# nv-tlabs/3dgrut

Measured on NVIDIA H100. Metric: train frames/sec (fwd+bwd render), higher is better.
Workload: dtype f32

## Files before the change

### 3dgrut_b200/csrc/gut_api.cu

```cuda
#include <cuda_runtime.h>

#include <algorithm>
#include <cmath>
#include <cstdarg>
#include <cstdio>
#include <cstdlib>
#include <cstring>
#include <new>
#include <string>

#include "gut_common.cuh"

using namespace gutb200;

namespace {


struct Quat {
    float w, x, y, z;
};
struct Mat3 {
    float m[3][3];
};
struct Pose {
    float t[3];
    Quat q;
};

Mat3 to_mat3(const Quat& q) {
    const float qxx = q.x * q.x, qyy = q.y * q.y, qzz = q.z * q.z;
    const float qxz = q.x * q.z, qxy = q.x * q.y, qyz = q.y * q.z;
    const float qwx = q.w * q.x, qwy = q.w * q.y, qwz = q.w * q.z;
    Mat3 r;
    r.m[0][0] = 1.f - 2.f * (qyy + qzz); r.m[0][1] = 2.f * (qxy + qwz); r.m[0][2] = 2.f * (qxz - qwy);
    r.m[1][0] = 2.f * (qxy - qwz); r.m[1][1] = 1.f - 2.f * (qxx + qzz); r.m[1][2] = 2.f * (qyz + qwx);
    r.m[2][0] = 2.f * (qxz + qwy); r.m[2][1] = 2.f * (qyz - qwx); r.m[2][2] = 1.f - 2.f * (qxx + qyy);
    return r;
}

Quat to_quat(const Mat3& a) {
    const float(*m)[3] = a.m;
    Quat q;
    const float tr = m[0][0] + m[1][1] + m[2][2];
    if (tr > 0.f) {
        const float S = std::sqrt(tr + 1.f) * 2.f;
        q = {0.25f * S, (m[1][2] - m[2][1]) / S, (m[2][0] - m[0][2]) / S, (m[0][1] - m[1][0]) / S};
    } else if (m[0][0] > m[1][1] && m[0][0] > m[2][2]) {
        const float S = std::sqrt(1.f + m[0][0] - m[1][1] - m[2][2]) * 2.f;
        q = {(m[1][2] - m[2][1]) / S, 0.25f * S, (m[1][0] + m[0][1]) / S, (m[2][0] + m[0][2]) / S};
    } else if (m[1][1] > m[2][2]) {
        const float S = std::sqrt(1.f + m[1][1] - m[0][0] - m[2][2]) * 2.f;
        q = {(m[2][0] - m[0][2]) / S, (m[1][0] + m[0][1]) / S, 0.25f * S, (m[2][1] + m[1][2]) / S};
    } else {
        const float S = std::sqrt(1.f + m[2][2] - m[0][0] - m[1][1]) * 2.f;
        q = {(m[0][1] - m[1][0]) / S, (m[2][0] + m[0][2]) / S, (m[2][1] + m[1][2]) / S, 0.25f * S};
    }
    return q;
}

Quat slerp(const Quat& x, const Quat& y, float t) {
    Quat z = y;
    float c = (x.w * y.w + x.x * y.x) + (x.y * y.y + x.z * y.z);
    if (c < 0.f) {
        z = {-y.w, -y.x, -y.y, -y.z};
        c = -c;
    }
    if (c > 1.f - 1.1920929e-07f) {
        const float a = 1.f - t;
        return {x.w * a + z.w * t, x.x * a + z.x * t, x.y * a + z.y * t, x.z * a + z.z * t};
    }
    const float ang = std::acos(c);
    const float s0 = std::sin((1.f - t) * ang), s1 = std::sin(t * ang), sd = std::sin(ang);
    return {(s0 * x.w + s1 * z.w) / sd, (s0 * x.x + s1 * z.x) / sd, (s0 * x.y + s1 * z.y) / sd, (s0 * x.z + s1 * z.z) / sd};
}

Pose pose_from7(const float* p) { return Pose{{p[0], p[1], p[2]}, Quat{p[6], p[3], p[4], p[5]}}; }

Pose pose_inverse(const Pose& p) {
    const Mat3 r = to_mat3(p.q);
    Mat3 inv;
    for (int c = 0; c < 3; ++c)
        for (int k = 0; k < 3; ++k) inv.m[c][k] = r.m[k][c];
    Pose o;
    o.q = to_quat(inv);
    for (int j = 0; j < 3; ++j) {
        float acc = 0.f;
        acc += (-1.0f * inv.m[0][j]) * p.t[0];
        acc += (-1.0f * inv.m[1][j]) * p.t[1];
        acc += (-1.0f * inv.m[2][j]) * p.t[2];
        o.t[j] = acc;
    }
    return o;
}

void pose_cols(const Pose& p, float cols[12]) {
    const Mat3 r = to_mat3(p.q);
    for (int c = 0; c < 3; ++c)
        for (int k = 0; k < 3; ++k) cols[c * 3 + k] = r.m[c][k];
    cols[9] = p.t[0];
    cols[10] = p.t[1];
    cols[11] = p.t[2];
}


struct DeviceBuffer {
    void* ptr = nullptr;
    size_t bytes = 0;
    cudaError_t reserve(size_t want, cudaStream_t s, bool zero = false) {
        if (want <= bytes) return cudaSuccess;
        if (ptr) {
            cudaError_t e = cudaFreeAsync(ptr, s);
            if (e != cudaSuccess) return e;
            ptr = nullptr;
            bytes = 0;
        }
        const size_t padded = (want + (want >> 3) + 255) & ~size_t(255);
        cudaError_t e = cudaMallocAsync(&ptr, padded, s);
        if (e != cudaSuccess) return e;
        bytes = padded;
        if (zero) e = cudaMemsetAsync(ptr, 0, padded, s);
        return e;
    }
    void release() {
        if (ptr) cudaFree(ptr);
        ptr = nullptr;
        bytes = 0;
    }
    template <typename T>
    T* as() const { return static_cast<T*>(ptr); }
};

}

struct gutb200_ctx {
    gutb200_config cfg;
    int device = 0;
    std::string error;
    cudaStream_t own_stream = nullptr;

    DeviceBuffer tiles_count, proj, depth, rgb, grad_acc;
    DeviceBuffer keys64, keys64_alt, vals_out, hit_words;
    DeviceBuffer tile_hist, tile_fill, sub_base, ranges, tile_order, chunk_base, totals, scan_parts;
    cudaEvent_t ev_total = nullptr;
    gutb200_camera fwd_camera{};
    DeviceBuffer h_particles, h_sph, h_rays_o, h_rays_d, h_rgba, h_dist, h_hits, h_vis, h_drgba, h_ddist, h_dpart, h_dsph;
    uint32_t* pinned_total = nullptr;

    FrameCamera cam{};
    FrameConfig fcfg{};
    int64_t n = -1, num_isect = 0, num_tiles = 0;
    bool have_forward = false;
    bool fwd_nht = false;
    cudaStream_t fwd_stream = nullptr;

    cudaEvent_t ev[4] = {nullptr, nullptr, nullptr, nullptr};
    double fwd_ms = 0, bwd_ms = 0;
    int fwd_calls = 0, bwd_calls = 0;
    bool fwd_pending = false, bwd_pending = false;
    int64_t launches = 0;

    cudaEvent_t st_ev[8][2] = {};
    bool st_pending[8] = {};
    double st_ms[8] = {};
    int st_calls[8] = {};
};

namespace {

int fail(gutb200_ctx* c, const char* fmt, ...) {
    char buf[512];
    va_list ap;
    va_start(ap, fmt);
    vsnprintf(buf, sizeof(buf), fmt, ap);
    va_end(ap);
    if (c) c->error = buf;
    return 1;
}

#define GUT_CUDA(ctx, expr)                                                                             \
    do {                                                                                                \
        cudaError_t e__ = (expr);                                                                       \
        if (e__ != cudaSuccess) return fail(ctx, "%s failed: %s", #expr, cudaGetErrorString(e__));      \
    } while (0)

void fill_frame(gutb200_ctx* c, const gutb200_camera* cam) {
    FrameCamera& f = c->cam;
    f.width = cam->width;
    f.height = cam->height;
    f.grid_x = (cam->width + kTile - 1) / kTile;
    f.grid_y = (cam->height + kTile - 1) / kTile;
    f.fx = cam->focal[0]; f.fy = cam->focal[1];
    f.cx = cam->principal[0]; f.cy = cam->principal[1];
    memcpy(f.radial, cam->radial, sizeof(f.radial));
    memcpy(f.tangential, cam->tangential, sizeof(f.tangential));
    memcpy(f.thin_prism, cam->thin_prism, sizeof(f.thin_prism));
    f.has_distortion = 0;
    for (float v : cam->radial) f.has_distortion |= (v != 0.f);
    for (float v : cam->tangential) f.has_distortion |= (v != 0.f);
    for (float v : cam->thin_prism) f.has_distortion |= (v != 0.f);
    f.res_x = static_cast<float>(cam->width);
    f.res_y = static_cast<float>(cam->height);
    f.model = cam->model;
    f.max_angle = cam->max_angle;
    f.ft_reference_poly = cam->ftheta_reference_poly;
    memcpy(f.ft_bw, cam->ftheta_bw, sizeof(f.ft_bw));
    memcpy(f.ft_fw, cam->ftheta_fw, sizeof(f.ft_fw));
    memcpy(f.ft_cde, cam->ftheta_cde, sizeof(f.ft_cde));
    const Pose ps = pose_from7(cam->pose_start), pe = pose_from7(cam->pose_end);
    const Mat3 rs = to_mat3(ps.q);
    for (int cc = 0; cc < 3; ++cc)
        for (int k = 0; k < 3; ++k) f.rot_start[cc * 3 + k] = rs.m[cc][k];
    for (int k = 0; k < 3; ++k) f.t_start[k] = ps.t[k];
    f.rolling_shutter = cam->rolling_shutter;
    f.rs_iterations = c->cfg.n_rolling_shutter_iterations;
    f.q_start[0] = ps.q.w; f.q_start[1] = ps.q.x; f.q_start[2] = ps.q.y; f.q_start[3] = ps.q.z;
    f.q_end[0] = pe.q.w; f.q_end[1] = pe.q.x; f.q_end[2] = pe.q.y; f.q_end[3] = pe.q.z;
    for (int k = 0; k < 3; ++k) f.t_end[k] = pe.t[k];
    Pose mid;
    mid.q = slerp(ps.q, pe.q, 0.5f);
    for (int k = 0; k < 3; ++k) mid.t[k] = ps.t[k] * (1.f - 0.5f) + pe.t[k] * 0.5f;
    const Pose inv = pose_inverse(mid);
    pose_cols(mid, f.view);
    pose_cols(inv, f.s2w);
    for (int k = 0; k < 3; ++k) f.cam_pos[k] = inv.t[k];

    FrameConfig& g = c->fcfg;
    const gutb200_config& s = c->cfg;
    g.kernel_degree = s.kernel_degree;
    g.min_kernel_density = s.min_kernel_density;
    g.min_alpha = s.min_alpha;
    g.max_alpha = s.max_alpha;
    g.min_transmittance = s.min_transmittance;
    g.ut_delta = s.ut_delta;
    g.ut_margin = s.ut_margin;
    const float D = 3.f;
    const float lambda = s.ut_alpha * s.ut_alpha * (D + s.ut_kappa) - D;
    g.w0_mean = lambda / (D + lambda);
    g.wi = 1.f / (2.f * (D + lambda));
    g.w0_cov = lambda / (D + lambda) + (1.f - s.ut_alpha * s.ut_alpha + s.ut_beta);
    g.rect_bounding = s.rect_bounding;
    g.tight_opacity_bounding = s.tight_opacity_bounding;
    g.tile_culling = s.tile_culling;
    g.global_z_order = s.global_z_order;
    g.subtile_culling = s.subtile_culling;
    g.k_buffer_size = s.k_buffer_size;
}

int check_args(gutb200_ctx* c, const gutb200_camera* cam, int64_t n, const void* particles, int32_t sph_degree) {
    if (!c) return 1;
    if (sph_degree < 0 || sph_degree > 3) return fail(c, "sph_degree %d out of range (0..3)", sph_degree);
    if (!cam || cam->width <= 0 || cam->height <= 0) return fail(c, "invalid camera resolution");
    if (cam->rolling_shutter < 0 || cam->rolling_shutter > 4) return fail(c, "rolling_shutter %d out of range (0 global, 1..4 readout directions)", cam->rolling_shutter);
    if (cam->model < 0 || cam->model > 2) return fail(c, "camera model %d unknown (0 = OpenCV pinhole, 1 = OpenCV fisheye, 2 = f-theta)", cam->model);
    if (n < 0 || n > 0x7FFFFFFF) return fail(c, "particle count %lld out of range", static_cast<long long>(n));
    if (reinterpret_cast<uintptr_t>(particles) & 15) return fail(c, "particle buffer must be 16-byte aligned");
    if (c->cfg.k_buffer_size < 0 || c->cfg.k_buffer_size > 16) return fail(c, "k_buffer_size %d out of range (0..16)", c->cfg.k_buffer_size);
    if (c->cfg.kernel_degree != 2 && c->cfg.kernel_degree != 4) return fail(c, "kernel_degree %d not built (2 or 4)", c->cfg.kernel_degree);
    if (((c->cfg.subtile_culling >> 4) & 3) == 3)
        return fail(c, "subtile_culling sub-block code 3 (bits 4-5) not built (0 = quarter-warps, 1 = half-warps, 2 = whole warps)");
    return 0;
}

struct StageTimer {
    gutb200_ctx* c;
    int id;
    cudaStream_t s;
    bool on;
    StageTimer(gutb200_ctx* ctx, int stage, cudaStream_t stream) : c(ctx), id(stage), s(stream), on(ctx->cfg.enable_timings >= 2) {
        if (on) {
            if (!c->st_ev[id][0]) {
                cudaEventCreate(&c->st_ev[id][0]);
                cudaEventCreate(&c->st_ev[id][1]);
            }
            cudaEventRecord(c->st_ev[id][0], s);
        }
    }
    ~StageTimer() {
        if (on) {
            cudaEventRecord(c->st_ev[id][1], s);
            c->st_pending[id] = true;
        }
    }
};

void drain_timers(gutb200_ctx* c) {
    float ms = 0.f;
    for (int i = 0; i < 8; ++i) {
        if (c->st_pending[i] && cudaEventSynchronize(c->st_ev[i][1]) == cudaSuccess &&
            cudaEventElapsedTime(&ms, c->st_ev[i][0], c->st_ev[i][1]) == cudaSuccess) {
            c->st_ms[i] += ms;
            c->st_calls[i]++;
        }
        c->st_pending[i] = false;
    }
    if (c->fwd_pending && cudaEventSynchronize(c->ev[1]) == cudaSuccess && cudaEventElapsedTime(&ms, c->ev[0], c->ev[1]) == cudaSuccess) {
        c->fwd_ms += ms;
        c->fwd_calls++;
    }
    c->fwd_pending = false;
    if (c->bwd_pending && cudaEventSynchronize(c->ev[3]) == cudaSuccess && cudaEventElapsedTime(&ms, c->ev[2], c->ev[3]) == cudaSuccess) {
        c->bwd_ms += ms;
        c->bwd_calls++;
    }
    c->bwd_pending = false;
}

}

extern "C" {

const char* gutb200_version(void) { return "3dgrut_b200 0.1 (sm_90a)"; }

void gutb200_default_config(gutb200_config* c) {
    c->kernel_degree = 2;
    c->min_kernel_density = 0.0113f;
    c->min_alpha = 1.0f / 255.0f;
    c->max_alpha = 0.99f;
    c->min_transmittance = 0.0001f;
    c->ut_alpha = 1.0f;
    c->ut_beta = 2.0f;
    c->ut_kappa = 0.0f;
    c->ut_delta = static_cast<float>(1.7320508075688772);
    c->ut_margin = 0.1f;
    c->rect_bounding = 1;
    c->tight_opacity_bounding = 1;
    c->tile_culling = 1;
    c->global_z_order = 1;
    c->enable_timings = 0;
    c->subtile_culling = 7;
    c->n_rolling_shutter_iterations = 5;
    c->k_buffer_size = 0;
    if (const char* e = std::getenv("GUTB200_SUBTILE_CULLING")) c->subtile_culling = std::atoi(e);
}

int gutb200_create(const gutb200_config* cfg, int device, gutb200_ctx** out) {
    if (!cfg || !out) return 1;
    *out = nullptr;
    int count = 0;
    if (cudaGetDeviceCount(&count) != cudaSuccess || count <= 0 || device < 0 || device >= count) return 2;
    gutb200_ctx* c = new (std::nothrow) gutb200_ctx();
    if (!c) return 3;
    c->cfg = *cfg;
    c->device = device;
    if (cudaSetDevice(device) != cudaSuccess || cudaStreamCreateWithFlags(&c->own_stream, cudaStreamNonBlocking) != cudaSuccess ||
        cudaMallocHost(reinterpret_cast<void**>(&c->pinned_total), 2 * sizeof(uint32_t)) != cudaSuccess ||
        cudaEventCreateWithFlags(&c->ev_total, cudaEventDisableTiming) != cudaSuccess) {
        delete c;
        return 4;
    }
    for (auto& e : c->ev) cudaEventCreate(&e);
    *out = c;
    return 0;
}

void gutb200_destroy(gutb200_ctx* c) {
    if (!c) return;
    cudaSetDevice(c->device);
    cudaDeviceSynchronize();
    DeviceBuffer* bufs[] = {&c->tiles_count, &c->proj, &c->depth, &c->rgb, &c->grad_acc, &c->keys64, &c->keys64_alt, &c->vals_out, &c->hit_words, &c->tile_hist,
                            &c->tile_fill, &c->scan_parts, &c->sub_base, &c->ranges, &c->tile_order, &c->chunk_base, &c->totals, &c->h_particles, &c->h_sph,
                            &c->h_rays_o, &c->h_rays_d, &c->h_rgba, &c->h_dist, &c->h_hits, &c->h_vis, &c->h_drgba, &c->h_ddist,
                            &c->h_dpart, &c->h_dsph};
    for (DeviceBuffer* b : bufs) b->release();
    if (c->pinned_total) cudaFreeHost(c->pinned_total);
    for (auto& e : c->ev)
        if (e) cudaEventDestroy(e);
    if (c->ev_total) cudaEventDestroy(c->ev_total);
    for (auto& pair : c->st_ev)
        for (auto& e : pair)
            if (e) cudaEventDestroy(e);
    if (c->own_stream) cudaStreamDestroy(c->own_stream);
    delete c;
}

const char* gutb200_last_error(const gutb200_ctx* c) { return c ? c->error.c_str() : "null context"; }

int64_t gutb200_launch_count(const gutb200_ctx* c) { return c ? c->launches : 0; }

}

namespace {

int check_nht_args(gutb200_ctx* c, const void* features, int32_t feature_dim, int32_t features_half) {
    if (feature_dim != 48) return fail(c, "NHT feature_dim %d not built (48 = 4 tetrahedron vertices x 12 features)", feature_dim);
    if (features_half != 0 && features_half != 1) return fail(c, "features_half must be 0 (fp32) or 1 (fp16), got %d", features_half);
    if (reinterpret_cast<uintptr_t>(features) & 15) return fail(c, "feature buffer must be 16-byte aligned");
    if (c->cfg.k_buffer_size > 0) return fail(c, "NHT features are not built with the k-buffer (k_buffer_size %d > 0)", c->cfg.k_buffer_size);
    return 0;
}

int forward_impl(gutb200_ctx* c, void* stream, const gutb200_camera* cam, int64_t n, const float* particles, const void* sph,
                 int32_t sph_degree, bool nht, bool half, const float* rays_o, const float* rays_d, float* out_rgba, float* out_dist,
                 float* out_hits, float* visibility) {
    cudaStream_t s = static_cast<cudaStream_t>(stream);
    GUT_CUDA(c, cudaSetDevice(c->device));
    c->have_forward = false;
    fill_frame(c, cam);
    const int64_t tiles = static_cast<int64_t>(c->cam.grid_x) * c->cam.grid_y;
    const size_t nn = static_cast<size_t>(n > 0 ? n : 1);

    if (c->cfg.enable_timings) {
        drain_timers(c);
        GUT_CUDA(c, cudaEventRecord(c->ev[0], s));
    }

    GUT_CUDA(c, c->tiles_count.reserve(nn * 4, s));
    GUT_CUDA(c, c->proj.reserve(nn * sizeof(ProjRecord), s));
    GUT_CUDA(c, c->depth.reserve(nn * 4, s));
    GUT_CUDA(c, c->rgb.reserve(nn * 12, s));
    const size_t tt = static_cast<size_t>(tiles);
    GUT_CUDA(c, c->tile_hist.reserve(tt * kTileSubs * 4, s));
    GUT_CUDA(c, c->tile_fill.reserve(tt * kTileSubs * 4, s));
    GUT_CUDA(c, c->sub_base.reserve(tt * kTileSubs * 4, s));
    GUT_CUDA(c, c->ranges.reserve(tt * 8, s));
    GUT_CUDA(c, c->tile_order.reserve(tt * 4, s));
    GUT_CUDA(c, c->chunk_base.reserve(tt * 4, s));
    GUT_CUDA(c, c->totals.reserve(16, s));
    GUT_CUDA(c, c->scan_parts.reserve(tile_scan_parts_words(static_cast<int>(tiles)) * 4, s));

    auto bin_and_render = [&](uint32_t capacity) -> int {
        {
            StageTimer t(c, 1, s);
            launch_tile_scan(s, static_cast<int>(tiles), c->tile_hist.as<uint32_t>(), capacity, c->ranges.as<uint32_t>(), c->sub_base.as<uint32_t>(),
                             c->chunk_base.as<uint32_t>(), c->tile_order.as<uint32_t>(), c->tile_fill.as<uint32_t>(), c->totals.as<uint32_t>(),
                             c->scan_parts.as<uint32_t>());
        }
        GUT_CUDA(c, cudaMemcpyAsync(c->pinned_total, c->totals.ptr, 2 * sizeof(uint32_t), cudaMemcpyDeviceToHost, s));
        GUT_CUDA(c, cudaEventRecord(c->ev_total, s));
        c->launches += 2;
        if (capacity > 0 && n > 0) {
            {
                StageTimer t(c, 2, s);
                launch_expand_place(s, c->cam, c->fcfg, n, c->proj.as<ProjRecord>(), c->depth.as<float>(), c->tile_hist.as<uint32_t>(),
                                    c->sub_base.as<uint32_t>(), c->totals.as<uint32_t>(), capacity, c->tile_fill.as<uint32_t>(),
                                    c->keys64.as<unsigned long long>());
            }
            {
                StageTimer t(c, 3, s);
                GUT_CUDA(c, launch_tile_sort(s, static_cast<int>(tiles), c->tile_order.as<uint32_t>(), c->ranges.as<uint32_t>(), c->totals.as<uint32_t>(),
                                             c->keys64.as<unsigned long long>(), c->keys64_alt.as<unsigned long long>(), c->vals_out.as<uint32_t>()));
            }
            c->launches += 2;
        }
        {
            StageTimer t(c, 5, s);
            if (c->fcfg.k_buffer_size == 0)
                GUT_CUDA(c, cudaMemsetAsync(c->hit_words.ptr, 0, hit_words_capacity(capacity, tiles) * 4, s));
            if (nht)
                launch_render_forward_nht(s, c->cam, c->fcfg, rays_o, rays_d, particles, sph, half, c->vals_out.as<uint32_t>(),
                                          c->ranges.as<uint32_t>(), c->tile_order.as<uint32_t>(), c->chunk_base.as<uint32_t>(),
                                          c->hit_words.as<uint32_t>(), out_rgba, out_dist, out_hits);
            else if (c->fcfg.k_buffer_size > 0)
                launch_render_forward_kbuffer(s, c->cam, c->fcfg, c->fcfg.k_buffer_size, rays_o, rays_d, particles, c->rgb.as<float>(),
                                              c->vals_out.as<uint32_t>(), c->ranges.as<uint32_t>(), out_rgba, out_dist, out_hits);
            else
                launch_render_forward(s, c->cam, c->fcfg, rays_o, rays_d, particles, c->rgb.as<float>(), c->vals_out.as<uint32_t>(),
                                      c->ranges.as<uint32_t>(), c->tile_order.as<uint32_t>(), c->chunk_base.as<uint32_t>(),
                                      c->hit_words.as<uint32_t>(), out_rgba, out_dist, out_hits);
        }
        c->launches++;
        return 0;
    };

    uint32_t total = 0;
    GUT_CUDA(c, cudaMemsetAsync(c->tile_hist.ptr, 0, tt * kTileSubs * 4, s));
    if (n > 0) {
        StageTimer t(c, 0, s);
        launch_project(s, c->cam, c->fcfg, n, particles, static_cast<const float*>(sph), sph_degree, c->tiles_count.as<uint32_t>(),
                       c->proj.as<ProjRecord>(), c->depth.as<float>(), c->rgb.as<float>(), visibility, c->tile_hist.as<uint32_t>(), !nht);
        c->launches++;
    }
    GUT_CUDA(c, c->vals_out.reserve(16, s));
    GUT_CUDA(c, c->hit_words.reserve(hit_words_capacity(0, tiles) * 4, s));
    uint32_t capacity = static_cast<uint32_t>(std::min<size_t>(std::min(c->keys64.bytes, c->keys64_alt.bytes) / 8, 0xFFFFFFF0u));
    capacity = static_cast<uint32_t>(std::min<size_t>(capacity, c->vals_out.bytes / 4));
    while (capacity > 0 && hit_words_capacity(capacity, tiles) * 4 > c->hit_words.bytes) capacity = capacity > 4096 ? capacity - 4096 : 0;
    if (int rc = bin_and_render(capacity)) return rc;
    GUT_CUDA(c, cudaEventSynchronize(c->ev_total));
    total = c->pinned_total[0];
    if (c->pinned_total[1] != 0u) {
        GUT_CUDA(c, c->keys64.reserve(static_cast<size_t>(total) * 8, s));
        GUT_CUDA(c, c->keys64_alt.reserve(static_cast<size_t>(total) * 8, s));
        GUT_CUDA(c, c->vals_out.reserve(static_cast<size_t>(total) * 4 + 16, s));
        GUT_CUDA(c, c->hit_words.reserve(hit_words_capacity(total + (total >> 3) + 64, tiles) * 4, s));
        capacity = total;
        if (int rc = bin_and_render(capacity)) return rc;
        GUT_CUDA(c, cudaEventSynchronize(c->ev_total));
        if (c->pinned_total[1] != 0u || c->pinned_total[0] != total) return fail(c, "internal error: intersection count changed between two passes");
    }
    GUT_CUDA(c, cudaGetLastError());
    if (c->cfg.enable_timings) {
        GUT_CUDA(c, cudaEventRecord(c->ev[1], s));
        c->fwd_pending = true;
    }
    c->n = n;
    c->num_isect = total;
    c->num_tiles = tiles;
    c->fwd_stream = s;
    c->fwd_camera = *cam;
    c->fwd_nht = nht;
    c->have_forward = true;
    return 0;
}

}

extern "C" {

int gutb200_forward(gutb200_ctx* c, void* stream, const gutb200_camera* cam, int64_t n, const float* particles, const float* sph,
                    int32_t sph_degree, const float* rays_o, const float* rays_d, float* out_rgba, float* out_dist, float* out_hits,
                    float* visibility) {
    if (int rc = check_args(c, cam, n, particles, sph_degree)) return rc;
    return forward_impl(c, stream, cam, n, particles, sph, sph_degree, false, false, rays_o, rays_d, out_rgba, out_dist, out_hits, visibility);
}

int gutb200_forward_nht(gutb200_ctx* c, void* stream, const gutb200_camera* cam, int64_t n, const float* particles, const void* features,
                        int32_t feature_dim, int32_t features_half, const float* rays_o, const float* rays_d, float* out_features_alpha,
                        float* out_dist, float* out_hits, float* visibility) {
    if (int rc = check_args(c, cam, n, particles, 0)) return rc;
    if (int rc = check_nht_args(c, features, feature_dim, features_half)) return rc;
    return forward_impl(c, stream, cam, n, particles, features, 0, true, features_half != 0, rays_o, rays_d, out_features_alpha, out_dist,
                        out_hits, visibility);
}

static int backward_impl(gutb200_ctx* c, void* stream, const gutb200_camera* cam, int64_t n, const float* particles, const void* sph,
                         int32_t sph_degree, bool nht, bool half, const float* rays_o, const float* rays_d, const float* out_rgba,
                         const float* d_rgba, const float* out_dist, const float* d_dist, float* d_particles, float* d_sph, bool compact) {
    cudaStream_t s = static_cast<cudaStream_t>(stream);
    if (!c->have_forward || c->fwd_stream != s || c->n != n || c->cam.width != cam->width || c->cam.height != cam->height)
        return fail(c, "backward needs the forward context of the same stream / particle count / resolution");
    if (memcmp(&c->fwd_camera, cam, sizeof(gutb200_camera)) != 0)
        return fail(c, "backward was called with a camera that differs from the immediately preceding forward's (poses / intrinsics)");
    if (c->fwd_nht != nht)
        return fail(c, nht ? "gutb200_backward_nht needs a gutb200_forward_nht before it (the preceding forward rendered SH radiance)"
                           : "the preceding forward rendered NHT features: its adjoint is gutb200_backward_nht");
    GUT_CUDA(c, cudaSetDevice(c->device));
    if (c->cfg.enable_timings) {
        GUT_CUDA(c, cudaEventRecord(c->ev[2], s));
    }
    const size_t nn = static_cast<size_t>(n > 0 ? n : 1);
    GUT_CUDA(c, c->grad_acc.reserve(nn * kGradRow * 4, s, true));
    if (nht && n > 0) GUT_CUDA(c, cudaMemsetAsync(d_sph, 0, static_cast<size_t>(n) * 48 * sizeof(float), s));
    if (c->num_isect > 0) {
        StageTimer t(c, 6, s);
        if (nht)
            GUT_CUDA(c, launch_render_backward_nht(s, c->cam, c->fcfg, rays_o, rays_d, particles, sph, half, c->vals_out.as<uint32_t>(),
                                                   c->ranges.as<uint32_t>(), c->tile_order.as<uint32_t>(), c->chunk_base.as<uint32_t>(),
                                                   c->hit_words.as<uint32_t>(), out_rgba, d_rgba, out_dist, d_dist, c->grad_acc.as<float>(),
                                                   d_sph));
        else if (c->fcfg.k_buffer_size > 0)
            launch_render_backward_kbuffer(s, c->cam, c->fcfg, c->fcfg.k_buffer_size, rays_o, rays_d, particles, c->rgb.as<float>(),
                                           c->vals_out.as<uint32_t>(), c->ranges.as<uint32_t>(), out_rgba, d_rgba, out_dist, d_dist,
                                           c->grad_acc.as<float>());
        else
            launch_render_backward(s, c->cam, c->fcfg, rays_o, rays_d, particles, c->rgb.as<float>(), c->vals_out.as<uint32_t>(),
                                   c->ranges.as<uint32_t>(), c->tile_order.as<uint32_t>(), c->chunk_base.as<uint32_t>(),
                                   c->hit_words.as<uint32_t>(), out_rgba, d_rgba, out_dist, d_dist, c->grad_acc.as<float>());
        c->launches++;
    }
    if (n > 0) {
        StageTimer t(c, 7, s);
        launch_project_backward(s, c->cam, n, particles, static_cast<const float*>(sph), sph_degree, c->rgb.as<float>(),
                                c->tiles_count.as<uint32_t>(), rays_o, c->grad_acc.as<float>(), d_particles, d_sph, compact,
                                c->fcfg.k_buffer_size == 0, !nht);
        c->launches++;
    }
    GUT_CUDA(c, cudaGetLastError());
    if (c->cfg.enable_timings) {
        GUT_CUDA(c, cudaEventRecord(c->ev[3], s));
        c->bwd_pending = true;
    }
    return 0;
}

int gutb200_backward(gutb200_ctx* c, void* stream, const gutb200_camera* cam, int64_t n, const float* particles, const float* sph,
                     int32_t sph_degree, const float* rays_o, const float* rays_d, const float* out_rgba, const float* d_rgba,
                     const float* out_dist, const float* d_dist, float* d_particles, float* d_sph) {
    if (int rc = check_args(c, cam, n, particles, sph_degree)) return rc;
    return backward_impl(c, stream, cam, n, particles, sph, sph_degree, false, false, rays_o, rays_d, out_rgba, d_rgba, out_dist, d_dist, d_particles,
                         d_sph, false);
}

int gutb200_backward_nht(gutb200_ctx* c, void* stream, const gutb200_camera* cam, int64_t n, const float* particles, const void* features,
                         int32_t feature_dim, int32_t features_half, const float* rays_o, const float* rays_d, const float* out_features_alpha,
                         const float* d_features_alpha, const float* out_dist, const float* d_dist, float* d_particles, float* d_features) {
    if (int rc = check_args(c, cam, n, particles, 0)) return rc;
    if (int rc = check_nht_args(c, features, feature_dim, features_half)) return rc;
    return backward_impl(c, stream, cam, n, particles, features, 0, true, features_half != 0, rays_o, rays_d, out_features_alpha, d_features_alpha,
                         out_dist, d_dist, d_particles, d_features, false);
}

int gutb200_backward_compact(gutb200_ctx* c, void* stream, const gutb200_camera* cam, int64_t n, const float* particles, const float* sph,
                             int32_t sph_degree, const float* rays_o, const float* rays_d, const float* out_rgba, const float* d_rgba,
                             const float* out_dist, const float* d_dist, float* d_particles, float* d_radiance) {
    if (int rc = check_args(c, cam, n, particles, sph_degree)) return rc;
    return backward_impl(c, stream, cam, n, particles, sph, sph_degree, false, false, rays_o, rays_d, out_rgba, d_rgba, out_dist, d_dist, d_particles,
                         d_radiance, true);
}

int gutb200_sph_grad_from_views(gutb200_ctx* c, void* stream, int64_t n, const float* particles, int32_t sph_degree, int32_t views,
                                const float* view_positions_host, const float* d_radiance_all, float* d_sph) {
    if (!c) return 1;
    if (views < 1 || views > 64) return fail(c, "views %d out of range (1..64)", views);
    if (n < 0 || !view_positions_host) return fail(c, "invalid arguments");
    if (sph_degree < 0 || sph_degree > 3) return fail(c, "sph_degree %d out of range", sph_degree);
    GUT_CUDA(c, cudaSetDevice(c->device));
    launch_sph_from_views(static_cast<cudaStream_t>(stream), n, particles, sph_degree, views, view_positions_host, d_radiance_all, d_sph);
    c->launches++;
    GUT_CUDA(c, cudaGetLastError());
    return 0;
}

int gutb200_camera_position(const gutb200_camera* cam, float* pos3) {
    if (!cam || !pos3) return 1;
    const Pose ps = pose_from7(cam->pose_start), pe = pose_from7(cam->pose_end);
    Pose mid;
    mid.q = slerp(ps.q, pe.q, 0.5f);
    for (int k = 0; k < 3; ++k) mid.t[k] = ps.t[k] * (1.f - 0.5f) + pe.t[k] * 0.5f;
    const Pose inv = pose_inverse(mid);
    for (int k = 0; k < 3; ++k) pos3[k] = inv.t[k];
    return 0;
}

int gutb200_forward_host(gutb200_ctx* c, const gutb200_camera* cam, int64_t n, const float* particles, const float* sph,
                         int32_t sph_degree, const float* rays_o, const float* rays_d, float* out_rgba, float* out_dist,
                         float* out_hits, float* visibility) {
    if (!c || !cam) return 1;
    cudaStream_t s = c->own_stream;
    const size_t np = static_cast<size_t>(n), px = static_cast<size_t>(cam->width) * cam->height;
    GUT_CUDA(c, cudaSetDevice(c->device));
    GUT_CUDA(c, c->h_particles.reserve(np * 48 + 16, s));
    GUT_CUDA(c, c->h_sph.reserve(np * 192 + 16, s));
    GUT_CUDA(c, c->h_rays_o.reserve(px * 12, s));
    GUT_CUDA(c, c->h_rays_d.reserve(px * 12, s));
    GUT_CUDA(c, c->h_rgba.reserve(px * 16, s));
    GUT_CUDA(c, c->h_dist.reserve(px * 4, s));
    GUT_CUDA(c, c->h_hits.reserve(px * 4, s));
    GUT_CUDA(c, c->h_vis.reserve(np * 4 + 16, s));
    GUT_CUDA(c, cudaMemcpyAsync(c->h_particles.ptr, particles, np * 48, cudaMemcpyHostToDevice, s));
    GUT_CUDA(c, cudaMemcpyAsync(c->h_sph.ptr, sph, np * 192, cudaMemcpyHostToDevice, s));
    GUT_CUDA(c, cudaMemcpyAsync(c->h_rays_o.ptr, rays_o, px * 12, cudaMemcpyHostToDevice, s));
    GUT_CUDA(c, cudaMemcpyAsync(c->h_rays_d.ptr, rays_d, px * 12, cudaMemcpyHostToDevice, s));
    if (int rc = gutb200_forward(c, s, cam, n, c->h_particles.as<float>(), c->h_sph.as<float>(), sph_degree, c->h_rays_o.as<float>(),
                                 c->h_rays_d.as<float>(), c->h_rgba.as<float>(), c->h_dist.as<float>(), c->h_hits.as<float>(),
                                 c->h_vis.as<float>()))
        return rc;
    GUT_CUDA(c, cudaMemcpyAsync(out_rgba, c->h_rgba.ptr, px * 16, cudaMemcpyDeviceToHost, s));
    GUT_CUDA(c, cudaMemcpyAsync(out_dist, c->h_dist.ptr, px * 4, cudaMemcpyDeviceToHost, s));
    GUT_CUDA(c, cudaMemcpyAsync(out_hits, c->h_hits.ptr, px * 4, cudaMemcpyDeviceToHost, s));
    if (np) GUT_CUDA(c, cudaMemcpyAsync(visibility, c->h_vis.ptr, np * 4, cudaMemcpyDeviceToHost, s));
    GUT_CUDA(c, cudaStreamSynchronize(s));
    return 0;
}

int gutb200_backward_host(gutb200_ctx* c, const gutb200_camera* cam, int64_t n, const float* particles, const float* sph,
                          int32_t sph_degree, const float* rays_o, const float* rays_d, const float* out_rgba, const float* d_rgba,
                          const float* out_dist, const float* d_dist, float* d_particles, float* d_sph) {
    if (!c || !cam) return 1;
    (void)particles; (void)sph; (void)rays_o; (void)rays_d;
    if (!c->have_forward || c->fwd_stream != c->own_stream)
        return fail(c, "backward needs the forward context of the same stream / particle count / resolution");
    cudaStream_t s = c->own_stream;
    const size_t np = static_cast<size_t>(n), px = static_cast<size_t>(cam->width) * cam->height;
    GUT_CUDA(c, cudaSetDevice(c->device));
    GUT_CUDA(c, c->h_drgba.reserve(px * 16, s));
    GUT_CUDA(c, c->h_ddist.reserve(px * 4, s));
    GUT_CUDA(c, c->h_dpart.reserve(np * 48 + 16, s));
    GUT_CUDA(c, c->h_dsph.reserve(np * 192 + 16, s));
    GUT_CUDA(c, cudaMemcpyAsync(c->h_rgba.ptr, out_rgba, px * 16, cudaMemcpyHostToDevice, s));
    GUT_CUDA(c, cudaMemcpyAsync(c->h_dist.ptr, out_dist, px * 4, cudaMemcpyHostToDevice, s));
    GUT_CUDA(c, cudaMemcpyAsync(c->h_drgba.ptr, d_rgba, px * 16, cudaMemcpyHostToDevice, s));
    GUT_CUDA(c, cudaMemcpyAsync(c->h_ddist.ptr, d_dist, px * 4, cudaMemcpyHostToDevice, s));
    if (int rc = gutb200_backward(c, s, cam, n, c->h_particles.as<float>(), c->h_sph.as<float>(), sph_degree, c->h_rays_o.as<float>(),
                                  c->h_rays_d.as<float>(), c->h_rgba.as<float>(), c->h_drgba.as<float>(), c->h_dist.as<float>(),
                                  c->h_ddist.as<float>(), c->h_dpart.as<float>(), c->h_dsph.as<float>()))
        return rc;
    if (np) {
        GUT_CUDA(c, cudaMemcpyAsync(d_particles, c->h_dpart.ptr, np * 48, cudaMemcpyDeviceToHost, s));
        GUT_CUDA(c, cudaMemcpyAsync(d_sph, c->h_dsph.ptr, np * 192, cudaMemcpyDeviceToHost, s));
    }
    GUT_CUDA(c, cudaStreamSynchronize(s));
    return 0;
}

int gutb200_last_stats(gutb200_ctx* c, int64_t* n, int64_t* num_intersections, int64_t* num_visible, int64_t* num_tiles) {
    if (!c || !c->have_forward) return fail(c, "no forward context");
    GUT_CUDA(c, cudaSetDevice(c->device));
    GUT_CUDA(c, cudaStreamSynchronize(c->fwd_stream));
    if (n) *n = c->n;
    if (num_intersections) *num_intersections = c->num_isect;
    if (num_tiles) *num_tiles = c->num_tiles;
    if (num_visible) {
        int64_t v = 0;
        if (c->n > 0) {
            uint32_t* h = new (std::nothrow) uint32_t[c->n];
            if (!h) return fail(c, "out of host memory");
            cudaError_t e = cudaMemcpy(h, c->tiles_count.ptr, static_cast<size_t>(c->n) * 4, cudaMemcpyDeviceToHost);
            for (int64_t i = 0; e == cudaSuccess && i < c->n; ++i) v += h[i] > 0;
            delete[] h;
            GUT_CUDA(c, e);
        }
        *num_visible = v;
    }
    return 0;
}

int gutb200_debug_copy(gutb200_ctx* c, int what, void* dst, size_t bytes) {
    if (!c || !c->have_forward) return fail(c, "no forward context");
    GUT_CUDA(c, cudaSetDevice(c->device));
    GUT_CUDA(c, cudaStreamSynchronize(c->fwd_stream));
    const void* src = nullptr;
    size_t have = 0;
    const size_t n = static_cast<size_t>(c->n), I = static_cast<size_t>(c->num_isect), T = static_cast<size_t>(c->num_tiles);
    switch (what) {
        case GUTB200_DBG_TILES_COUNT: src = c->tiles_count.ptr; have = n * 4; break;
        case GUTB200_DBG_SORTED_KEYS: {
            if (bytes != I * 8) return fail(c, "debug buffer %d holds %zu bytes, caller asked for %zu", what, I * 8, bytes);
            if (I == 0) return 0;
            void* tmp = nullptr;
            GUT_CUDA(c, cudaMalloc(&tmp, I * 8));
            launch_synth_tile_keys(c->fwd_stream, static_cast<int>(T), c->ranges.as<uint32_t>(), c->vals_out.as<uint32_t>(), c->depth.as<float>(),
                                   static_cast<uint64_t*>(tmp));
            cudaError_t e = cudaStreamSynchronize(c->fwd_stream);
            if (e == cudaSuccess) e = cudaMemcpy(dst, tmp, I * 8, cudaMemcpyDeviceToHost);
            cudaFree(tmp);
            GUT_CUDA(c, e);
            return 0;
        }
        case GUTB200_DBG_SORTED_VALUES: src = c->vals_out.ptr; have = I * 4; break;
        case GUTB200_DBG_TILE_RANGES: src = c->ranges.ptr; have = T * 8; break;
        case GUTB200_DBG_DEPTH: src = c->depth.ptr; have = n * 4; break;
        case GUTB200_DBG_RGB: src = c->rgb.ptr; have = n * 12; break;
        case GUTB200_DBG_PROJ: src = c->proj.ptr; have = n * sizeof(ProjRecord); break;
        default: return fail(c, "unknown debug buffer %d", what);
    }
    if (bytes != have) return fail(c, "debug buffer %d holds %zu bytes, caller asked for %zu", what, have, bytes);
    if (have) GUT_CUDA(c, cudaMemcpy(dst, src, have, cudaMemcpyDeviceToHost));
    return 0;
}

int gutb200_debug_work_counters(gutb200_ctx* c, const float* particles, const float* rays_o, const float* rays_d, uint64_t* counters16) {
    if (!c || !c->have_forward) return fail(c, "no forward context");
    if (c->fcfg.k_buffer_size != 0) return fail(c, "work counters exist for the unsorted path (k_buffer_size 0) only");
    if (c->fwd_nht) return fail(c, "work counters exist for the SH radiance forward only");
    GUT_CUDA(c, cudaSetDevice(c->device));
    cudaStream_t s = c->fwd_stream;
    unsigned long long* dctr = nullptr;
    GUT_CUDA(c, cudaMalloc(&dctr, 128));
    cudaMemsetAsync(dctr, 0, 128, s);
    for (int i = 0; i < 16; ++i) counters16[i] = 0;
    if (c->num_isect > 0)
        launch_count_work(s, c->cam, c->fcfg, rays_o, rays_d, particles, c->rgb.as<float>(), c->vals_out.as<uint32_t>(), c->ranges.as<uint32_t>(),
                          c->tile_order.as<uint32_t>(), c->chunk_base.as<uint32_t>(), c->hit_words.as<uint32_t>(), dctr);
    cudaError_t e = cudaStreamSynchronize(s);
    if (e == cudaSuccess) e = cudaMemcpy(counters16, dctr, 128, cudaMemcpyDeviceToHost);
    cudaFree(dctr);
    GUT_CUDA(c, e);
    return 0;
}

int gutb200_debug_fma_peak(gutb200_ctx* c, int repeats, float* tflops) {
    if (!c || !tflops) return 1;
    GUT_CUDA(c, cudaSetDevice(c->device));
    cudaDeviceProp prop;
    GUT_CUDA(c, cudaGetDeviceProperties(&prop, c->device));
    const int blocks = prop.multiProcessorCount * 8, iters = 2048;
    float* sink = nullptr;
    GUT_CUDA(c, cudaMalloc(&sink, 4));
    cudaEvent_t a, b;
    cudaEventCreate(&a);
    cudaEventCreate(&b);
    float best = 0.f;
    for (int r = 0; r < repeats + 1; ++r) {
        cudaEventRecord(a, c->own_stream);
        launch_fma_peak(c->own_stream, blocks, iters, sink);
        cudaEventRecord(b, c->own_stream);
        cudaEventSynchronize(b);
        float ms = 0.f;
        cudaEventElapsedTime(&ms, a, b);
        const double flops = static_cast<double>(blocks) * 256.0 * iters * 16.0 * 8.0 * 2.0;
        if (r > 0 && ms > 0.f) best = fmaxf(best, static_cast<float>(flops / (ms * 1e-3) / 1e12));
    }
    cudaEventDestroy(a);
    cudaEventDestroy(b);
    cudaFree(sink);
    *tflops = best;
    GUT_CUDA(c, cudaGetLastError());
    return 0;
}

int gutb200_set_timings(gutb200_ctx* c, int level) {
    if (!c) return 1;
    drain_timers(c);
    c->cfg.enable_timings = level;
    return 0;
}

int gutb200_collect_stage_times(gutb200_ctx* c, float* mean_ms ) {
    if (!c || !mean_ms) return 1;
    drain_timers(c);
    for (int i = 0; i < 8; ++i) {
        mean_ms[i] = c->st_calls[i] ? static_cast<float>(c->st_ms[i] / c->st_calls[i]) : 0.f;
        c->st_ms[i] = 0;
        c->st_calls[i] = 0;
    }
    return 0;
}

int gutb200_collect_times(gutb200_ctx* c, float* forward_ms, float* backward_ms) {
    if (!c) return 1;
    drain_timers(c);
    if (forward_ms) *forward_ms = c->fwd_calls ? static_cast<float>(c->fwd_ms / c->fwd_calls) : 0.f;
    if (backward_ms) *backward_ms = c->bwd_calls ? static_cast<float>(c->bwd_ms / c->bwd_calls) : 0.f;
    c->fwd_ms = c->bwd_ms = 0;
    c->fwd_calls = c->bwd_calls = 0;
    return 0;
}

}
```

### 3dgrut_b200/csrc/gut_binning.cu

```cuda
#include <cstdlib>

#include "gut_common.cuh"

namespace gutb200 {

namespace {

constexpr unsigned kFullMask = 0xFFFFFFFFu;


constexpr int kScanTiles = 256;
constexpr int kScanBuckets = 34;
constexpr int kScanPart = 2 + kScanBuckets;

__device__ __forceinline__ uint32_t tile_count(const uint32_t* __restrict__ counts, int t, uint4 v[4]) {
    const uint4* c4 = reinterpret_cast<const uint4*>(counts + static_cast<size_t>(t) * kTileSubs);
    v[0] = c4[0]; v[1] = c4[1]; v[2] = c4[2]; v[3] = c4[3];
    return (v[0].x + v[0].y + v[0].z + v[0].w) + (v[1].x + v[1].y + v[1].z + v[1].w) + (v[2].x + v[2].y + v[2].z + v[2].w) +
           (v[3].x + v[3].y + v[3].z + v[3].w);
}

__device__ __forceinline__ void scan_pair(uint32_t a, uint32_t b, uint32_t& ex_a, uint32_t& ex_b, uint32_t& tot_a, uint32_t& tot_b) {
    __shared__ uint32_t w_a[kScanTiles / 32], w_b[kScanTiles / 32];
    const int lane = threadIdx.x & 31, warp = threadIdx.x >> 5;
    uint32_t ia = a, ib = b;
#pragma unroll
    for (int o = 1; o < 32; o <<= 1) {
        const uint32_t x = __shfl_up_sync(kFullMask, ia, o), y = __shfl_up_sync(kFullMask, ib, o);
        if (lane >= o) {
            ia += x;
            ib += y;
        }
    }
    if (lane == 31) {
        w_a[warp] = ia;
        w_b[warp] = ib;
    }
    __syncthreads();
    uint32_t ra = 0, rb = 0;
    tot_a = 0;
    tot_b = 0;
#pragma unroll
    for (int w = 0; w < kScanTiles / 32; ++w) {
        if (w == warp) {
            ra = tot_a;
            rb = tot_b;
        }
        tot_a += w_a[w];
        tot_b += w_b[w];
    }
    ex_a = ra + ia - a;
    ex_b = rb + ib - b;
}

__global__ void __launch_bounds__(kScanTiles) tile_scan_reduce_kernel(int num_tiles, const uint32_t* __restrict__ counts,
                                                                      uint32_t* __restrict__ parts) {
    static_assert(kTileSubs == 16, "a tile's sub-counters are four 16-byte loads");
    __shared__ uint32_t hist[kScanBuckets];
    if (threadIdx.x < kScanBuckets) hist[threadIdx.x] = 0;
    __syncthreads();
    const int t = blockIdx.x * kScanTiles + threadIdx.x, lane = threadIdx.x & 31;
    const bool live = t < num_tiles;
    uint4 v[4];
    const uint32_t c = live ? tile_count(counts, t, v) : 0u;
    const int bucket = live ? __clz(c) + 1 : 64 + lane;
    const unsigned peers = __match_any_sync(kFullMask, bucket);
    if (live && (peers & ((1u << lane) - 1u)) == 0u) atomicAdd(&hist[bucket], static_cast<uint32_t>(__popc(peers)));
    uint32_t ex_n, ex_c, tot_n, tot_c;
    scan_pair(c, (c + 31u) >> 5, ex_n, ex_c, tot_n, tot_c);
    uint32_t* p = parts + static_cast<size_t>(blockIdx.x) * kScanPart;
    if (threadIdx.x == 0) {
        p[0] = tot_n;
        p[1] = tot_c;
    }
    if (threadIdx.x < kScanBuckets) p[2 + threadIdx.x] = hist[threadIdx.x];
}

__global__ void __launch_bounds__(kScanTiles) tile_scan_write_kernel(int num_tiles, const uint32_t* __restrict__ counts, uint32_t capacity,
                                                                     const uint32_t* __restrict__ parts, uint32_t* __restrict__ ranges,
                                                                     uint32_t* __restrict__ sub_base, uint32_t* __restrict__ chunk_base,
                                                                     uint32_t* __restrict__ order, uint32_t* __restrict__ fill,
                                                                     uint32_t* __restrict__ totals) {
    __shared__ uint32_t s_before[kScanPart], s_all[kScanPart];
    __shared__ uint32_t hist[kScanBuckets];
    const int t = blockIdx.x * kScanTiles + threadIdx.x, lane = threadIdx.x & 31;
    if (threadIdx.x < kScanPart) {
        uint32_t before = 0, all = 0;
        for (int b = 0; b < static_cast<int>(gridDim.x); ++b) {
            const uint32_t x = parts[static_cast<size_t>(b) * kScanPart + threadIdx.x];
            before += b < static_cast<int>(blockIdx.x) ? x : 0u;
            all += x;
        }
        s_before[threadIdx.x] = before;
        s_all[threadIdx.x] = all;
    }
    __syncthreads();
    if (threadIdx.x == 0) {
        uint32_t run = 0;
        for (int b = 1; b < kScanBuckets; ++b) {
            hist[b] = run + s_before[2 + b];
            run += s_all[2 + b];
        }
    }
    const uint32_t total = s_all[0];
    const bool overflow = total > capacity;
    if (blockIdx.x == 0 && threadIdx.x == 0) {
        totals[0] = total;
        totals[1] = overflow ? 1u : 0u;
    }
    const bool live = t < num_tiles;
    uint4 v[4];
    const uint32_t c = live ? tile_count(counts, t, v) : 0u;
    uint32_t ex_n, ex_c, tot_n, tot_c;
    scan_pair(c, (c + 31u) >> 5, ex_n, ex_c, tot_n, tot_c);
    if (live) {
        uint32_t r = s_before[0] + ex_n;
        const uint32_t first = r;
        uint4 b[4];
#pragma unroll
        for (int q = 0; q < 4; ++q) {
            b[q].x = r; r += v[q].x; b[q].y = r; r += v[q].y; b[q].z = r; r += v[q].z; b[q].w = r; r += v[q].w;
        }
        uint4* sb = reinterpret_cast<uint4*>(sub_base + static_cast<size_t>(t) * kTileSubs);
        sb[0] = b[0]; sb[1] = b[1]; sb[2] = b[2]; sb[3] = b[3];
        const uint32_t fill0 = overflow ? 0xC0000000u : 0u;
        const uint4 fill4 = make_uint4(fill0, fill0, fill0, fill0);
        uint4* fl = reinterpret_cast<uint4*>(fill + static_cast<size_t>(t) * kTileSubs);
        fl[0] = fill4; fl[1] = fill4; fl[2] = fill4; fl[3] = fill4;
        reinterpret_cast<uint2*>(ranges)[t] = (overflow || c == 0u) ? make_uint2(0u, 0u) : make_uint2(first, r);
        chunk_base[t] = overflow ? 0u : s_before[1] + ex_c;
    }
    const int bucket = live ? __clz(c) + 1 : 64 + lane;
    const unsigned peers = __match_any_sync(kFullMask, bucket);
    const int leader = __ffs(peers) - 1;
    uint32_t slot = 0;
    if (live && lane == leader) slot = atomicAdd(&hist[bucket], static_cast<uint32_t>(__popc(peers)));
    slot = __shfl_sync(kFullMask, slot, leader);
    if (live) order[slot + __popc(peers & ((1u << lane) - 1u))] = static_cast<uint32_t>(t);
}



constexpr int kSortThreads = 512, kSortWarps = kSortThreads / 32;
constexpr int kSortUnroll = 4;
constexpr int kStageKeys = 4096, kStagePerLane = kStageKeys / kSortThreads;

__device__ __forceinline__ bool scan_digits(uint32_t (*s_cnt)[256], uint32_t* s_tot, int* s_flag, int aw, uint32_t n) {
    const int lane = threadIdx.x & 31, warp = threadIdx.x >> 5, d = threadIdx.x;
    uint32_t tot = 0, incl = 0;
    if (d < 256) {
        for (int w = 0; w < aw; ++w) tot += s_cnt[w][d];
        if (tot == n) *s_flag = 1;
        incl = tot;
#pragma unroll
        for (int o = 1; o < 32; o <<= 1) {
            const uint32_t v = __shfl_up_sync(kFullMask, incl, o);
            if (lane >= o) incl += v;
        }
        if (lane == 31) s_tot[warp] = incl;
    }
    __syncthreads();
    const bool skip = *s_flag != 0;
    if (!skip && d < 256) {
        uint32_t run = incl - tot;
        for (int w = 0; w < warp; ++w) run += s_tot[w];
        for (int w = 0; w < aw; ++w) {
            const uint32_t c = s_cnt[w][d];
            s_cnt[w][d] = run;
            run += c;
        }
    }
    __syncthreads();
    return skip;
}

template <bool BALLOT>
__device__ __forceinline__ uint32_t rank_key(uint32_t* cnt_row, unsigned long long k, int shift, bool have) {
    const int lane = threadIdx.x & 31;
    const uint32_t dg = have ? (static_cast<uint32_t>(k >> shift) & 255u) : 256u + lane;
    unsigned peers;
    if (BALLOT) {
        peers = __ballot_sync(kFullMask, have);
#pragma unroll
        for (int b = 0; b < 8; ++b) {
            const bool bit = (dg >> b) & 1u;
            const unsigned bal = __ballot_sync(kFullMask, bit);
            peers &= bit ? bal : ~bal;
        }
        if (!have) peers = 1u << lane;
    } else {
        peers = __match_any_sync(kFullMask, dg);
    }
    const int leader = __ffs(peers) - 1;
    uint32_t slot = 0;
    if (have && lane == leader) slot = atomicAdd(&cnt_row[dg], static_cast<uint32_t>(__popc(peers)));
    slot = __shfl_sync(kFullMask, slot, leader);
    return slot + __popc(peers & ((1u << lane) - 1u));
}

__device__ __forceinline__ void fix_equal_depth_runs(unsigned long long* a, uint32_t n) {
    for (uint32_t i = threadIdx.x; i + 1 < n; i += kSortThreads) {
        const unsigned long long x = a[i];
        if ((x >> 32) != (a[i + 1] >> 32)) continue;
        if (i > 0 && (a[i - 1] >> 32) == (x >> 32)) continue;
        uint32_t e = i + 2;
        while (e < n && (a[e] >> 32) == (x >> 32)) ++e;
        for (uint32_t p = i + 1; p < e; ++p) {
            const unsigned long long k = a[p];
            uint32_t q = p;
            while (q > i && a[q - 1] > k) {
                a[q] = a[q - 1];
                --q;
            }
            a[q] = k;
        }
    }
}

template <bool BALLOT>
__global__ void __launch_bounds__(kSortThreads) tile_sort_kernel(const uint32_t* __restrict__ order, const uint32_t* __restrict__ ranges,
                                                                 const uint32_t* __restrict__ totals, unsigned long long* keys,
                                                                 unsigned long long* keys_alt, uint32_t* __restrict__ sorted_values) {
    __shared__ uint32_t s_cnt[kSortWarps][256];
    __shared__ uint32_t s_tot[8];
    __shared__ int s_flag;
    extern __shared__ unsigned long long s_keys[];
    if (totals[1] != 0u) return;
    const uint32_t tile = order[blockIdx.x];
    const uint32_t begin = ranges[tile * 2], n = ranges[tile * 2 + 1] - begin;
    if (n == 0u) return;
    const int lane = threadIdx.x & 31, warp = threadIdx.x >> 5;
    unsigned long long* src = keys + begin;
    unsigned long long* dst = keys_alt + begin;
    const int aw = static_cast<int>(min(static_cast<uint32_t>(kSortWarps), max(1u, (n + 127u) / 128u)));
    const uint32_t seg = ((n + aw - 1) / aw + 31u) & ~31u;
    const uint32_t w0 = min(n, warp * seg), w1 = min(n, w0 + seg);

    if (n <= static_cast<uint32_t>(kStageKeys)) {
        for (uint32_t i = threadIdx.x; i < n; i += kSortThreads) s_keys[i] = src[i];
        for (int shift = 32; shift < 64; shift += 8) {
            for (int i = threadIdx.x; i < aw * 256; i += kSortThreads) (&s_cnt[0][0])[i] = 0u;
            if (threadIdx.x == 0) s_flag = 0;
            __syncthreads();
            unsigned long long k[kStagePerLane];
#pragma unroll
            for (int u = 0; u < kStagePerLane; ++u) {
                const uint32_t i = w0 + u * 32 + lane;
                k[u] = i < w1 ? s_keys[i] : 0ull;
                if (i < w1) atomicAdd(&s_cnt[warp][static_cast<uint32_t>(k[u] >> shift) & 255u], 1u);
            }
            __syncthreads();
            if (scan_digits(s_cnt, s_tot, &s_flag, aw, n)) continue;
#pragma unroll
            for (int u = 0; u < kStagePerLane; ++u) {
                if (w0 + u * 32 >= w1) break;
                const bool have = w0 + u * 32 + lane < w1;
                const uint32_t slot = rank_key<BALLOT>(s_cnt[warp], k[u], shift, have);
                if (have) s_keys[slot] = k[u];
            }
            __syncthreads();
        }
        fix_equal_depth_runs(s_keys, n);
        __syncthreads();
        for (uint32_t i = threadIdx.x; i < n; i += kSortThreads) sorted_values[begin + i] = static_cast<uint32_t>(s_keys[i]);
        return;
    }

    for (int shift = 32; shift < 64; shift += 8) {
        for (int i = threadIdx.x; i < aw * 256; i += kSortThreads) (&s_cnt[0][0])[i] = 0u;
        if (threadIdx.x == 0) s_flag = 0;
        __syncthreads();
        for (uint32_t i0 = w0; i0 < w1; i0 += 32 * kSortUnroll) {
            unsigned long long k[kSortUnroll];
#pragma unroll
            for (int u = 0; u < kSortUnroll; ++u) {
                const uint32_t i = i0 + u * 32 + lane;
                k[u] = i < w1 ? src[i] : ~0ull;
            }
#pragma unroll
            for (int u = 0; u < kSortUnroll; ++u)
                if (i0 + u * 32 + lane < w1) atomicAdd(&s_cnt[warp][static_cast<uint32_t>(k[u] >> shift) & 255u], 1u);
        }
        __syncthreads();
        if (scan_digits(s_cnt, s_tot, &s_flag, aw, n)) continue;
        for (uint32_t i0 = w0; i0 < w1; i0 += 32 * kSortUnroll) {
            unsigned long long k[kSortUnroll];
#pragma unroll
            for (int u = 0; u < kSortUnroll; ++u) {
                const uint32_t i = i0 + u * 32 + lane;
                k[u] = i < w1 ? src[i] : 0ull;
            }
#pragma unroll
            for (int u = 0; u < kSortUnroll; ++u) {
                if (i0 + u * 32 >= w1) break;
                const bool have = i0 + u * 32 + lane < w1;
                const uint32_t slot = rank_key<BALLOT>(s_cnt[warp], k[u], shift, have);
                if (have) dst[slot] = k[u];
            }
        }
        __syncthreads();
        unsigned long long* t = src;
        src = dst;
        dst = t;
    }
    fix_equal_depth_runs(src, n);
    __syncthreads();
    for (uint32_t i = threadIdx.x; i < n; i += kSortThreads) sorted_values[begin + i] = static_cast<uint32_t>(src[i]);
}

__global__ void __launch_bounds__(256) synth_tile_keys_kernel(const uint32_t* __restrict__ ranges, const uint32_t* __restrict__ vals,
                                                              const float* __restrict__ depth, uint64_t* __restrict__ out) {
    const uint32_t tile = blockIdx.x;
    const uint32_t begin = ranges[tile * 2], end = ranges[tile * 2 + 1];
    for (uint32_t k = begin + threadIdx.x; k < end; k += blockDim.x)
        out[k] = (static_cast<uint64_t>(tile) << 32) | __float_as_uint(depth[vals[k]]);
}

}

size_t tile_scan_parts_words(int num_tiles) { return static_cast<size_t>(max(1, (num_tiles + kScanTiles - 1) / kScanTiles)) * kScanPart; }

void launch_tile_scan(cudaStream_t s, int num_tiles, const uint32_t* counts, uint32_t capacity, uint32_t* ranges, uint32_t* sub_base,
                      uint32_t* chunk_base, uint32_t* order, uint32_t* fill, uint32_t* totals, uint32_t* parts) {
    const int blocks = max(1, (num_tiles + kScanTiles - 1) / kScanTiles);
    tile_scan_reduce_kernel<<<blocks, kScanTiles, 0, s>>>(num_tiles, counts, parts);
    tile_scan_write_kernel<<<blocks, kScanTiles, 0, s>>>(num_tiles, counts, capacity, parts, ranges, sub_base, chunk_base, order, fill, totals);
}

cudaError_t launch_tile_sort(cudaStream_t s, int num_tiles, const uint32_t* order, const uint32_t* ranges, const uint32_t* totals,
                             unsigned long long* keys, unsigned long long* keys_alt, uint32_t* sorted_values) {
    if (num_tiles <= 0) return cudaSuccess;
    static const bool use_match = [] { const char* e = std::getenv("GUTB200_SORT_MATCH"); return e && std::atoi(e) != 0; }();
    constexpr size_t kStageBytes = kStageKeys * sizeof(unsigned long long);
    static const cudaError_t opt_in = [] {
        cudaError_t e = cudaFuncSetAttribute(tile_sort_kernel<false>, cudaFuncAttributeMaxDynamicSharedMemorySize, static_cast<int>(kStageBytes));
        if (e == cudaSuccess)
            e = cudaFuncSetAttribute(tile_sort_kernel<true>, cudaFuncAttributeMaxDynamicSharedMemorySize, static_cast<int>(kStageBytes));
        return e;
    }();
    if (opt_in != cudaSuccess) return opt_in;
    if (use_match)
        tile_sort_kernel<false><<<num_tiles, kSortThreads, kStageBytes, s>>>(order, ranges, totals, keys, keys_alt, sorted_values);
    else
        tile_sort_kernel<true><<<num_tiles, kSortThreads, kStageBytes, s>>>(order, ranges, totals, keys, keys_alt, sorted_values);
    return cudaGetLastError();
}

void launch_synth_tile_keys(cudaStream_t s, int num_tiles, const uint32_t* ranges, const uint32_t* vals, const float* depth, uint64_t* out) {
    if (num_tiles <= 0) return;
    synth_tile_keys_kernel<<<num_tiles, 256, 0, s>>>(ranges, vals, depth, out);
}

}
```

### 3dgrut_b200/csrc/gut_common.cuh

```cuda
#pragma once
#include <cuda_runtime.h>
#include <stdint.h>

#include "../../include/gut_b200.h"

namespace gutb200 {

constexpr int kTile         = 16;
constexpr int kTilePixels   = kTile * kTile;
constexpr uint32_t kInvalid = 0xFFFFFFFFu;

struct FrameCamera {
    int width, height, grid_x, grid_y;
    float fx, fy, cx, cy;
    float radial[6], tangential[2], thin_prism[4];
    float rot_start[9];
    float t_start[3];
    float view[12];
    float s2w[12];
    float cam_pos[3];
    float res_x, res_y;
    int has_distortion;
    int model;
    float max_angle;
    int ft_reference_poly;
    float ft_bw[6], ft_fw[6], ft_cde[3];
    int rolling_shutter, rs_iterations;
    float q_start[4], q_end[4], t_end[3];
};

struct FrameConfig {
    int kernel_degree;
    float min_kernel_density, min_alpha, max_alpha, min_transmittance;
    float ut_delta, ut_margin;
    float w0_mean, wi, w0_cov;
    int rect_bounding, tight_opacity_bounding, tile_culling, global_z_order;
    int subtile_culling;
    int k_buffer_size;
};

struct __align__(16) ProjRecord {
    float cx, cy, ex, ey;
    float ca, cb, cc, op;
};

constexpr int kGradRow = 20;

void launch_project(cudaStream_t s, const FrameCamera& cam, const FrameConfig& cfg, int64_t n, const float* particles,
                    const float* sph, int sph_degree, uint32_t* tiles_count, ProjRecord* proj, float* depth, float* rgb,
                    float* visibility, uint32_t* tile_hist, bool radiance = true);
void launch_expand_place(cudaStream_t s, const FrameCamera& cam, const FrameConfig& cfg, int64_t n, const ProjRecord* proj, const float* depth,
                         const uint32_t* tile_hist, const uint32_t* sub_base, const uint32_t* totals, uint32_t capacity, uint32_t* fill,
                         unsigned long long* keys);
constexpr int kTileSubs = 16;
size_t tile_scan_parts_words(int num_tiles);
void launch_tile_scan(cudaStream_t s, int num_tiles, const uint32_t* counts, uint32_t capacity, uint32_t* ranges, uint32_t* sub_base,
                      uint32_t* chunk_base, uint32_t* order, uint32_t* fill, uint32_t* totals, uint32_t* parts);
cudaError_t launch_tile_sort(cudaStream_t s, int num_tiles, const uint32_t* order, const uint32_t* ranges, const uint32_t* totals,
                             unsigned long long* keys, unsigned long long* keys_alt, uint32_t* sorted_values);
void launch_synth_tile_keys(cudaStream_t s, int num_tiles, const uint32_t* ranges, const uint32_t* vals, const float* depth, uint64_t* out);

inline size_t hit_words_capacity(int64_t num_isect, int64_t tiles) { return (static_cast<size_t>(num_isect) / 32 + static_cast<size_t>(tiles) + 1) * 32; }
void launch_render_forward(cudaStream_t s, const FrameCamera& cam, const FrameConfig& cfg, const float* rays_o,
                           const float* rays_d, const float* particles, const float* rgb, const uint32_t* sorted_values,
                           const uint32_t* ranges, const uint32_t* tile_order, const uint32_t* chunk_base, uint32_t* hit_words, float* out_rgba,
                           float* out_dist, float* out_hits);
void launch_count_work(cudaStream_t s, const FrameCamera& cam, const FrameConfig& cfg, const float* rays_o, const float* rays_d,
                       const float* particles, const float* rgb, const uint32_t* sorted_values, const uint32_t* ranges,
                       const uint32_t* tile_order, const uint32_t* chunk_base, uint32_t* hit_words, unsigned long long* counters8);
void launch_render_backward(cudaStream_t s, const FrameCamera& cam, const FrameConfig& cfg, const float* rays_o,
                            const float* rays_d, const float* particles, const float* rgb, const uint32_t* sorted_values,
                            const uint32_t* ranges, const uint32_t* tile_order, const uint32_t* chunk_base, const uint32_t* hit_words,
                            const float* out_rgba, const float* d_rgba, const float* out_dist, const float* d_dist, float* grad_acc);
void launch_render_forward_nht(cudaStream_t s, const FrameCamera& cam, const FrameConfig& cfg, const float* rays_o, const float* rays_d,
                               const float* particles, const void* features, bool half, const uint32_t* sorted_values, const uint32_t* ranges,
                               const uint32_t* tile_order, const uint32_t* chunk_base, uint32_t* hit_words, float* out_features_alpha,
                               float* out_dist, float* out_hits);
cudaError_t launch_render_backward_nht(cudaStream_t s, const FrameCamera& cam, const FrameConfig& cfg, const float* rays_o, const float* rays_d,
                                       const float* particles, const void* features, bool half, const uint32_t* sorted_values,
                                       const uint32_t* ranges, const uint32_t* tile_order, const uint32_t* chunk_base, const uint32_t* hit_words,
                                       const float* out_features_alpha, const float* d_features_alpha, const float* out_dist, const float* d_dist,
                                       float* grad_acc, float* d_features);
void launch_fma_peak(cudaStream_t s, int blocks, int iters, float* sink);
void launch_render_forward_kbuffer(cudaStream_t s, const FrameCamera& cam, const FrameConfig& cfg, int K, const float* rays_o, const float* rays_d,
                                   const float* particles, const float* rgb, const uint32_t* sorted_values, const uint32_t* ranges,
                                   float* out_rgba, float* out_dist, float* out_hits);
void launch_render_backward_kbuffer(cudaStream_t s, const FrameCamera& cam, const FrameConfig& cfg, int K, const float* rays_o, const float* rays_d,
                                    const float* particles, const float* rgb, const uint32_t* sorted_values, const uint32_t* ranges,
                                    const float* out_rgba, const float* d_rgba, const float* out_dist, const float* d_dist, float* grad_acc);
void launch_project_backward(cudaStream_t s, const FrameCamera& cam, int64_t n, const float* particles, const float* sph,
                             int sph_degree, const float* rgb, const uint32_t* tiles_count, const float* rays_o, float* grad_acc,
                             float* d_particles, float* d_sph, bool compact, bool canon, bool radiance = true);
void launch_sph_from_views(cudaStream_t s, int64_t n, const float* particles, int sph_degree, int views, const float* view_positions,
                           const float* d_radiance_all, float* d_sph);

size_t sort32_temp_bytes(int64_t n);
void run_sort32_pairs(cudaStream_t s, void* temp, size_t temp_bytes, const uint32_t* kin, uint32_t* kout, const uint32_t* vin,
                      uint32_t* vout, int64_t n, int end_bit);

}
```

### 3dgrut_b200/csrc/gut_render.cu

```cuda
#include "gut_common.cuh"
#include "hit_math.cuh"
#include "render_tile.cuh"
#include "subtile_cull.cuh"
#include "tma.cuh"

namespace gutb200 {

namespace {

constexpr int kBatch = 256;



struct FwdSmem : FwdRecords<kBatch> {
    float4 col[kBatch];
};

struct RadiancePayload {
    float4* col;
    const float* __restrict__ rgb;
    float cr = 0.f, cg = 0.f, cb = 0.f;
    __device__ __forceinline__ void entry(int slot, uint32_t idx) {
        col[slot] = make_float4(fmaxf(rgb[idx * 3 + 0], 0.f), fmaxf(rgb[idx * 3 + 1], 0.f), fmaxf(rgb[idx * 3 + 2], 0.f), 0.f);
    }
    __device__ __forceinline__ void batch(const uint32_t* __restrict__, uint32_t, int, int) {}
    __device__ __forceinline__ void add(int j, float w, float, float, float) {
        const float4 c = col[j];
        cr += c.x * w;
        cg += c.y * w;
        cb += c.z * w;
    }
};

template <int DEG, bool COUNT>
__global__ void __launch_bounds__(kTilePixels) render_forward_kernel(FrameCamera cam, FrameConfig cfg,
                                                                     const float* __restrict__ rays_o,
                                                                     const float* __restrict__ rays_d,
                                                                     const float* __restrict__ particles,
                                                                     const float* __restrict__ rgb,
                                                                     const uint32_t* __restrict__ sorted_values,
                                                                     const uint32_t* __restrict__ ranges,
                                                                     const uint32_t* __restrict__ tile_order,
                                                                     const uint32_t* __restrict__ chunk_base, uint32_t* __restrict__ hit_words,
                                                                     float* __restrict__ out_rgba, float* __restrict__ out_dist,
                                                                     float* __restrict__ out_hits, WorkCounters* __restrict__ ctr) {
    __shared__ FwdSmem sm;
    const int tid = threadIdx.x;
    const TileRay tr = tile_ray(cam, rays_o, rays_d, tile_order, tid);
    RadiancePayload pay{sm.col, rgb};
    float T = 1.f, dist = 0.f;
    uint32_t hits = 0;
    forward_list<DEG, COUNT>(cam, cfg, sm, pay, tr, tid, rays_o, particles, sorted_values, ranges, chunk_base, hit_words, T, dist, hits, ctr);
    if (COUNT) return;

    const int64_t pix = tr.pix;
    if (tr.valid) {
        reinterpret_cast<float4*>(out_rgba)[pix] = make_float4(pay.cr, pay.cg, pay.cb, 1.0f - T);
        out_dist[pix] = dist;
        out_hits[pix] = static_cast<float>(hits);
    } else if (tr.inside) {
        reinterpret_cast<float4*>(out_rgba)[pix] = make_float4(0.f, 0.f, 0.f, 0.f);
        out_dist[pix] = 1e06f;
        out_hits[pix] = 0.f;
    }
}


struct BwdSmem : BwdRecords<kBatch> {
    float4 cl[kBatch];
    uint32_t hw[(kBatch / 32) * kWordsPerChunk];
    float4 rows[kTilePixels / 32][32 * kGradRow / 4];
};

template <int SUBL>
__device__ __forceinline__ int sub_first(int lane) { return SUBL == 32 ? 0 : SUBL == 16 ? (lane & 4) : (lane & 20); }

template <int SUBL>
__device__ __forceinline__ int sub_lane(int first, int i) {
    if (SUBL == 32) return i;
    if (SUBL == 16) return first | (i & 3) | ((i & 12) << 1);
    return first | (i & 3) | ((i & 4) << 1);
}

template <int SUBL>
__device__ __forceinline__ int sub_rank(int lane) {
    if (SUBL == 32) return lane;
    if (SUBL == 16) return (lane & 3) | ((lane >> 1) & 12);
    return (lane & 3) | ((lane >> 1) & 4);
}


struct BwdRay {
    float Cix, Ciy, Ciz, Cgx, Cgy, Cgz, Tint, Tgrad, Dint, Dgrad;
    float T, Cx, Cy, Cz, D;
};

struct RadianceHit {
    static constexpr int kDepthSlot = 16;
    static constexpr bool kHitPoint = false;
    float4 cl;
    __device__ __forceinline__ void at_hit(const BwdSmem& sm, int j, const BwdRay&, float, float, float, float, float (&)[19]) { cl = sm.cl[j]; }
    __device__ __forceinline__ float common(const FrameConfig&, BwdRay& st, float T, float weight, float inv_next, float, float partial,
                                            float (&g)[19]) {
        g[13] = st.Cgx * weight; g[14] = st.Cgy * weight; g[15] = st.Cgz * weight;
        st.Cx += weight * cl.x; st.Cy += weight * cl.y; st.Cz += weight * cl.z;
        const float rcx = fmaxf((st.Cix - st.Cx) * inv_next, 0.f);
        const float rcy = fmaxf((st.Ciy - st.Cy) * inv_next, 0.f);
        const float rcz = fmaxf((st.Ciz - st.Cz) * inv_next, 0.f);
        return partial + T * ((cl.x - rcx) * st.Cgx + (cl.y - rcy) * st.Cgy + (cl.z - rcz) * st.Cgz);
    }
};

template <int DEG, bool FAST, int SUBL>
__device__ __forceinline__ void backward_tile(const FrameConfig& cfg, BwdSmem& sm, const Ray& ray, float ofx, float ofy, float ofz, int tid,
                                              int lane, uint32_t begin, uint32_t end, const float* __restrict__ particles,
                                              const float* __restrict__ rgb, const uint32_t* __restrict__ sorted_values,
                                              const uint32_t* __restrict__ hit_words, bool use_words, bool alive, BwdRay& st,
                                              float* __restrict__ grad_acc) {
    const float dox = ray.ox - ofx, doy = ray.oy - ofy, doz = ray.oz - ofz;
    const bool depth_grads = __any_sync(kFull, alive && (st.Dgrad != 0.f));
    const int quarter = lane_quarter(lane);
    const unsigned sub_lanes = SUBL == 32 ? kFull : SUBL == 16 ? (quarter_lanes(quarter & 1) | quarter_lanes((quarter & 1) | 2)) : quarter_lanes(quarter);
    const int first = sub_first<SUBL>(lane);
    const int col = sub_rank<SUBL>(lane);
    const int cols = depth_grads ? 5 : 4;
    float4* rows = sm.rows[tid >> 5];
    backward_batches<FAST>(sm, sm.hw, ofx, ofy, ofz, tid, begin, end, particles, sorted_values, hit_words, use_words, alive,
        [&](uint32_t idx) {
            sm.cl[tid] = make_float4(fmaxf(rgb[idx * 3 + 0], 0.f), fmaxf(rgb[idx * 3 + 1], 0.f), fmaxf(rgb[idx * 3 + 2], 0.f), __uint_as_float(idx));
        },
        [](uint32_t, int) {},
        [&](int count) {
        for (int c = 0; c < count; c += 32) {
            if (__all_sync(kFull, !alive)) break;
            const uint32_t* hw = sm.hw + (c >> 5) * kWordsPerChunk + (tid >> 5) * 4;
            unsigned todo;
            if (SUBL == 32) todo = hw[0] | hw[1] | hw[2] | hw[3];
            else if (SUBL == 16) todo = hw[quarter & 1] | hw[(quarter & 1) | 2];
            else todo = hw[quarter];
            if (count - c < 32) todo &= (1u << (count - c)) - 1u;
            while (__any_sync(kFull, todo != 0u)) {
                const bool act = todo != 0u;
                const int j = act ? c + __ffs(todo) - 1 : c;
                todo &= todo - 1;
                float g[19];
#pragma unroll
                for (int i = 0; i < 19; ++i) g[i] = 0.f;
                bool hit = false;
                if (act && alive) hit = backward_pair<DEG, FAST, RadianceHit>(cfg, sm, j, ray, dox, doy, doz, depth_grads, st, alive, g);
                const unsigned hits = __ballot_sync(kFull, hit);
                if (hits) {
                    float4* mine = rows + lane * (kGradRow / 4);
                    mine[0] = make_float4(g[0], g[1], g[2], g[3]);
                    mine[1] = make_float4(g[4], g[5], g[6], g[7]);
                    mine[2] = make_float4(g[8], g[9], g[10], g[11]);
                    mine[3] = make_float4(g[12], g[13], g[14], g[15]);
                    if (depth_grads) mine[4] = make_float4(g[16], g[17], g[18], 0.f);
                    __syncwarp();
                    if ((hits & sub_lanes) && col < cols) {
                        float4 s = rows[sub_lane<SUBL>(first, 0) * (kGradRow / 4) + col];
#pragma unroll
                        for (int i = 1; i < SUBL; ++i) {
                            const float4 v = rows[sub_lane<SUBL>(first, i) * (kGradRow / 4) + col];
                            s.x += v.x; s.y += v.y; s.z += v.z; s.w += v.w;
                        }
                        atomicAdd(reinterpret_cast<float4*>(grad_acc + static_cast<size_t>(__float_as_uint(sm.cl[j].w)) * kGradRow) + col, s);
                    }
                    __syncwarp();
                    if (__all_sync(kFull, !alive)) break;
                }
            }
        }
    });
}

template <int DEG, int SUBL>
__global__ void __launch_bounds__(kTilePixels, 3) render_backward_kernel(FrameCamera cam, FrameConfig cfg,
                                                                      const float* __restrict__ rays_o,
                                                                      const float* __restrict__ rays_d,
                                                                      const float* __restrict__ particles,
                                                                      const float* __restrict__ rgb,
                                                                      const uint32_t* __restrict__ sorted_values,
                                                                      const uint32_t* __restrict__ ranges,
                                                                      const uint32_t* __restrict__ tile_order,
                                                                      const uint32_t* __restrict__ chunk_base,
                                                                      const uint32_t* __restrict__ hit_words,
                                                                      const float* __restrict__ out_rgba, const float* __restrict__ d_rgba,
                                                                      const float* __restrict__ out_dist, const float* __restrict__ d_dist,
                                                                      float* __restrict__ grad_acc) {
    __shared__ BwdSmem sm;
    const int tid = threadIdx.x;
    const TileRay tr = tile_ray(cam, rays_o, rays_d, tile_order, tid);
    const int64_t pix = tr.pix;

    BwdRay st;
    st.Cix = st.Ciy = st.Ciz = st.Cgx = st.Cgy = st.Cgz = 0.f;
    st.Tint = 1.f; st.Tgrad = 0.f; st.Dint = 0.f; st.Dgrad = 0.f;
    st.T = 1.f; st.Cx = st.Cy = st.Cz = st.D = 0.f;
    if (tr.valid) {
        const float4 o = reinterpret_cast<const float4*>(out_rgba)[pix];
        const float4 g = reinterpret_cast<const float4*>(d_rgba)[pix];
        st.Cix = o.x; st.Ciy = o.y; st.Ciz = o.z;
        st.Cgx = g.x; st.Cgy = g.y; st.Cgz = g.z;
        st.Tint = 1.f - o.w;
        st.Tgrad = -1.f * g.w;
        st.Dint = out_dist[pix];
        st.Dgrad = d_dist[pix];
    }

    float ofx, ofy, ofz;
    const bool fast = frame_common_origin(cam, rays_o, tr.inside, pix, ofx, ofy, ofz);
    const uint32_t begin = ranges[tr.tile * 2], end = ranges[tr.tile * 2 + 1];
    const uint32_t* words = hit_words + static_cast<size_t>(chunk_base[tr.tile]) * kWordsPerChunk;
    const bool use_words = (cfg.subtile_culling & 4) != 0;
    if (fast)
        backward_tile<DEG, true, SUBL>(cfg, sm, tr.ray, ofx, ofy, ofz, tid, tid & 31, begin, end, particles, rgb, sorted_values, words, use_words, tr.valid, st, grad_acc);
    else
        backward_tile<DEG, false, SUBL>(cfg, sm, tr.ray, ofx, ofy, ofz, tid, tid & 31, begin, end, particles, rgb, sorted_values, words, use_words, tr.valid, st, grad_acc);
}


constexpr float kC1 = 0.4886025119029199f;
__constant__ float kC2[5] = {1.0925484305920792f, -1.0925484305920792f, 0.31539156525252005f, -1.0925484305920792f,
                             0.5462742152960396f};
__constant__ float kC3[7] = {-0.5900435899266435f, 2.890611442640554f, -0.4570457994644658f, 0.3731763325901154f,
                             -0.4570457994644658f, 1.445305721320277f,  -0.5900435899266435f};

constexpr int kPbThreads = 128;
constexpr int kAccVec = kGradRow / 4;
constexpr uint32_t kAccBytes = kGradRow * 4;

template <bool COMPACT, bool CANON, bool SPH>
__global__ void __launch_bounds__(kPbThreads) project_backward_kernel(FrameCamera cam, int64_t n, const float* __restrict__ particles,
                                                                      const float* __restrict__ sph, int deg, const float* __restrict__ rgb,
                                                                      const uint32_t* __restrict__ tiles_count, const float* __restrict__ rays_o,
                                                                      float* __restrict__ grad_acc, float* __restrict__ d_particles,
                                                                      float* __restrict__ d_sph) {
    __shared__ __align__(128) float4 s_acc[kPbThreads * kAccVec];
    __shared__ __align__(128) float4 s_sh[kPbThreads * 12];
    __shared__ __align__(128) float4 s_dp[kPbThreads * 3];
    __shared__ __align__(8) uint64_t s_bar;
    const int tid = threadIdx.x;
    const int64_t base = static_cast<int64_t>(blockIdx.x) * kPbThreads;
    const int cnt = static_cast<int>(min(static_cast<int64_t>(kPbThreads), n - base));
    if (tid == 0) {
        mbar_init(&s_bar, kPbThreads);
        fence_proxy_async();
    }
    __syncthreads();
    const int64_t i = base + tid;
    const bool in_range = tid < cnt;
    const bool vis = in_range && (tiles_count[i] != 0u);
    const bool want_sh = SPH && vis && (deg > 0);
    mbar_expect_tx(&s_bar, (tid == 0 ? static_cast<uint32_t>(cnt) * kAccBytes : 0u) + (want_sh ? 192u : 0u));
    if (tid == 0) tma_bulk_g2s(s_acc, grad_acc + base * kGradRow, static_cast<uint32_t>(cnt) * kAccBytes, &s_bar);
    if (want_sh) tma_bulk_g2s(s_sh + tid * 12, sph + i * 48, 192u, &s_bar);
    float4 p = make_float4(0.f, 0.f, 0.f, 0.f), pq = p, ps = p;
    float c0 = 0.f, c1 = 0.f, c2 = 0.f;
    if (vis) {
        p = __ldg(reinterpret_cast<const float4*>(particles + i * 12));
        if (CANON) {
            pq = __ldg(reinterpret_cast<const float4*>(particles + i * 12) + 1);
            ps = __ldg(reinterpret_cast<const float4*>(particles + i * 12) + 2);
        }
        if (SPH) { c0 = rgb[i * 3 + 0]; c1 = rgb[i * 3 + 1]; c2 = rgb[i * 3 + 2]; }
    }
    float ofx = 0.f, ofy = 0.f, ofz = 0.f;
    if (CANON) {
        const float ax = rays_o[0], ay = rays_o[1], az = rays_o[2];
        const float* m = cam.s2w;
        ofx = m[0] * ax + m[3] * ay + m[6] * az + m[9];
        ofy = m[1] * ax + m[4] * ay + m[7] * az + m[10];
        ofz = m[2] * ax + m[5] * ay + m[8] * az + m[11];
    }
    mbar_wait(&s_bar, 0);

    const float4 zero = make_float4(0.f, 0.f, 0.f, 0.f);
    if (in_range) {
        float4 a0 = s_acc[tid * kAccVec + 0], a1 = s_acc[tid * kAccVec + 1], a2 = s_acc[tid * kAccVec + 2];
        float4 a3 = s_acc[tid * kAccVec + 3];
        const float4 a4 = s_acc[tid * kAccVec + 4];
#pragma unroll
        for (int k = 0; k < kAccVec; ++k) s_acc[tid * kAccVec + k] = zero;
        if (CANON) {
            const float w00 = a1.x, w01 = a1.y, w02 = a1.z, w10 = a1.w, w11 = a2.x, w12 = a2.y, w20 = a2.z, w21 = a2.w, w22 = a3.x;
            a3 = make_float4(a3.y, a3.z, a3.w, 0.f);
            a1 = zero;
            a2 = zero;
            if (vis) {
                const float r = pq.x, x = pq.y, y = pq.z, z = pq.w;
                const float xx = x * x, yy = y * y, zz = z * z, xy = x * y, xz = x * z, yz = y * z;
                const float rx = r * x, ry = r * y, rz = r * z;
                const float r0x = 1.f - 2.f * (yy + zz), r0y = 2.f * (xy + rz), r0z = 2.f * (xz - ry);
                const float r1x = 2.f * (xy - rz), r1y = 1.f - 2.f * (xx + zz), r1z = 2.f * (yz + rx);
                const float r2x = 2.f * (xz + ry), r2y = 2.f * (yz - rx), r2z = 1.f - 2.f * (xx + yy);
                const float isx = 1.0f / ps.x, isy = 1.0f / ps.y, isz = 1.0f / ps.z;
                const float pcx = ofx - p.x, pcy = ofy - p.y, pcz = ofz - p.z;
                const float gox = isx * (r0x * pcx + r0y * pcy + r0z * pcz);
                const float goy = isy * (r1x * pcx + r1y * pcy + r1z * pcz);
                const float goz = isz * (r2x * pcx + r2y * pcy + r2z * pcz);
                const float prx = isx * a0.x, pry = isy * a0.y, prz = isz * a0.z;
                a0.x = -(prx * r0x + pry * r1x + prz * r2x);
                a0.y = -(prx * r0y + pry * r1y + prz * r2y);
                a0.z = -(prx * r0z + pry * r1z + prz * r2z);
                a2.x = a4.x - isx * isx * (r0x * w00 + r0y * w01 + r0z * w02) - gox * prx;
                a2.y = a4.y - isy * isy * (r1x * w10 + r1y * w11 + r1z * w12) - goy * pry;
                a2.z = a4.z - isz * isz * (r2x * w20 + r2y * w21 + r2z * w22) - goz * prz;
                const float m00 = isx * w00 + prx * pcx, m01 = isx * w01 + prx * pcy, m02 = isx * w02 + prx * pcz;
                const float m10 = isy * w10 + pry * pcx, m11 = isy * w11 + pry * pcy, m12 = isy * w12 + pry * pcz;
                const float m20 = isz * w20 + prz * pcx, m21 = isz * w21 + prz * pcy, m22 = isz * w22 + prz * pcz;
                a1.x = 2.f * (z * (m01 - m10) + y * (m20 - m02) + x * (m12 - m21));
                a1.y = 2.f * (y * (m01 + m10) + z * (m02 + m20) + r * (m12 - m21)) - 4.f * x * (m11 + m22);
                a1.z = 2.f * (x * (m01 + m10) + r * (m20 - m02) + z * (m12 + m21)) - 4.f * y * (m00 + m22);
                a1.w = 2.f * (r * (m01 - m10) + x * (m02 + m20) + y * (m12 + m21)) - 4.f * z * (m00 + m11);
            }
        }
        float dpx = a0.x, dpy = a0.y, dpz = a0.z;
        float4* row = s_sh + tid * 12;
        if (!SPH) {
        } else if (!vis) {
#pragma unroll
            for (int k = 0; k < 12; ++k) row[k] = zero;
        } else {
            const float vx = p.x - cam.cam_pos[0], vy = p.y - cam.cam_pos[1], vz = p.z - cam.cam_pos[2];
            const float len = sqrtf(vx * vx + vy * vy + vz * vz);
            const float inv_len = len > 0.f ? 1.0f / len : 0.f;
            const float x = len > 0.f ? vx * inv_len : 1.f, y = vy * inv_len, z = vz * inv_len;
            const float mgr = c0 > 0.f ? a3.x : 0.f, mgg = c1 > 0.f ? a3.y : 0.f, mgb = c2 > 0.f ? a3.z : 0.f;
            float bs[16];
            sh_basis16(deg, x, y, z, bs);
            if (deg > 0 && len > 0.f) {
                float cf[48];
#pragma unroll
                for (int k = 0; k < 12; ++k) {
                    const float4 v = row[k];
                    cf[k * 4] = v.x; cf[k * 4 + 1] = v.y; cf[k * 4 + 2] = v.z; cf[k * 4 + 3] = v.w;
                }
                float sc[16];
#pragma unroll
                for (int k = 0; k < 16; ++k) sc[k] = cf[k * 3] * mgr + cf[k * 3 + 1] * mgg + cf[k * 3 + 2] * mgb;
                const float xx = x * x, yy = y * y, zz = z * z, xy = x * y, yz = y * z, xz = x * z;
                float gx = -kC1 * sc[3], gy = -kC1 * sc[1], gz = kC1 * sc[2];
                if (deg > 1) {
                    gx += kC2[0] * y * sc[4] + kC2[2] * (-2.f * x) * sc[6] + kC2[3] * z * sc[7] + kC2[4] * (2.f * x) * sc[8];
                    gy += kC2[0] * x * sc[4] + kC2[1] * z * sc[5] + kC2[2] * (-2.f * y) * sc[6] + kC2[4] * (-2.f * y) * sc[8];
                    gz += kC2[1] * y * sc[5] + kC2[2] * (4.f * z) * sc[6] + kC2[3] * x * sc[7];
                    if (deg > 2) {
                        gx += kC3[0] * (6.f * xy) * sc[9] + kC3[1] * yz * sc[10] + kC3[2] * (-2.f * xy) * sc[11] + kC3[3] * (-6.f * xz) * sc[12] +
                              kC3[4] * (4.f * zz - 3.f * xx - yy) * sc[13] + kC3[5] * (2.f * xz) * sc[14] + kC3[6] * (3.f * xx - 3.f * yy) * sc[15];
                        gy += kC3[0] * (3.f * xx - 3.f * yy) * sc[9] + kC3[1] * xz * sc[10] + kC3[2] * (4.f * zz - xx - 3.f * yy) * sc[11] +
                              kC3[3] * (-6.f * yz) * sc[12] + kC3[4] * (-2.f * xy) * sc[13] + kC3[5] * (-2.f * yz) * sc[14] +
                              kC3[6] * (-6.f * xy) * sc[15];
                        gz += kC3[1] * xy * sc[10] + kC3[2] * (8.f * yz) * sc[11] + kC3[3] * (6.f * zz - 3.f * xx - 3.f * yy) * sc[12] +
                              kC3[4] * (8.f * xz) * sc[13] + kC3[5] * (xx - yy) * sc[14];
                    }
                }
                const float dd = x * gx + y * gy + z * gz;
                dpx += (gx - x * dd) * inv_len;
                dpy += (gy - y * dd) * inv_len;
                dpz += (gz - z * dd) * inv_len;
            }
            if (COMPACT) {
                row[0] = make_float4(mgr, mgg, mgb, 0.f);
            } else {
                float o[48];
#pragma unroll
                for (int k = 0; k < 16; ++k) {
                    o[k * 3 + 0] = bs[k] * mgr;
                    o[k * 3 + 1] = bs[k] * mgg;
                    o[k * 3 + 2] = bs[k] * mgb;
                }
#pragma unroll
                for (int k = 0; k < 12; ++k) row[k] = make_float4(o[k * 4], o[k * 4 + 1], o[k * 4 + 2], o[k * 4 + 3]);
            }
        }
        s_dp[tid * 3 + 0] = make_float4(dpx, dpy, dpz, a0.w);
        s_dp[tid * 3 + 1] = a1;
        s_dp[tid * 3 + 2] = make_float4(a2.x, a2.y, a2.z, 0.f);
    }
    if (SPH && COMPACT) {
        const float4 mine = in_range ? s_sh[tid * 12] : zero;
        __syncthreads();
        s_sh[tid] = mine;
    }
    fence_proxy_async();
    __syncthreads();
    if (tid == 0) {
        if (SPH && COMPACT)
            tma_bulk_s2g(d_sph + base * 4, s_sh, static_cast<uint32_t>(cnt) * 16u);
        else if (SPH)
            tma_bulk_s2g(d_sph + base * 48, s_sh, static_cast<uint32_t>(cnt) * 192u);
        tma_bulk_s2g(d_particles + base * 12, s_dp, static_cast<uint32_t>(cnt) * 48u);
        tma_bulk_s2g(grad_acc + base * kGradRow, s_acc, static_cast<uint32_t>(cnt) * kAccBytes);
        tma_commit_group();
        tma_wait_group_read0();
    }
}

struct ViewPositions {
    float pos[64][3];
};

__global__ void __launch_bounds__(128) sph_from_views_kernel(int64_t n, const float* __restrict__ particles, int deg, int views, ViewPositions vp,
                                                              const float4* __restrict__ d_radiance_all, float4* __restrict__ d_sph) {
    const int64_t i = static_cast<int64_t>(blockIdx.x) * blockDim.x + threadIdx.x;
    if (i >= n) return;
    const float4 p = __ldg(reinterpret_cast<const float4*>(particles + i * 12));
    float o[48];
#pragma unroll
    for (int k = 0; k < 48; ++k) o[k] = 0.f;
    for (int v = 0; v < views; ++v) {
        const float4 g = __ldg(d_radiance_all + static_cast<int64_t>(v) * n + i);
        if (g.x == 0.f && g.y == 0.f && g.z == 0.f) continue;
        const float vx = p.x - vp.pos[v][0], vy = p.y - vp.pos[v][1], vz = p.z - vp.pos[v][2];
        const float len = sqrtf(vx * vx + vy * vy + vz * vz);
        const float inv_len = len > 0.f ? 1.0f / len : 0.f;
        const float x = len > 0.f ? vx * inv_len : 1.f, y = vy * inv_len, z = vz * inv_len;
        float bs[16];
        sh_basis16(deg, x, y, z, bs);
#pragma unroll
        for (int k = 0; k < 16; ++k) {
            o[k * 3 + 0] += bs[k] * g.x;
            o[k * 3 + 1] += bs[k] * g.y;
            o[k * 3 + 2] += bs[k] * g.z;
        }
    }
    float4* row = d_sph + i * 12;
#pragma unroll
    for (int k = 0; k < 12; ++k) row[k] = make_float4(o[k * 4], o[k * 4 + 1], o[k * 4 + 2], o[k * 4 + 3]);
}

}

void launch_render_forward(cudaStream_t s, const FrameCamera& cam, const FrameConfig& cfg, const float* rays_o,
                           const float* rays_d, const float* particles, const float* rgb, const uint32_t* sorted_values,
                           const uint32_t* ranges, const uint32_t* tile_order, const uint32_t* chunk_base, uint32_t* hit_words, float* out_rgba,
                           float* out_dist, float* out_hits) {
    const unsigned grid = cam.grid_x * cam.grid_y;
    if (cfg.kernel_degree == 4)
        render_forward_kernel<4, false><<<grid, kTilePixels, 0, s>>>(cam, cfg, rays_o, rays_d, particles, rgb, sorted_values, ranges, tile_order, chunk_base, hit_words, out_rgba, out_dist, out_hits, nullptr);
    else
        render_forward_kernel<2, false><<<grid, kTilePixels, 0, s>>>(cam, cfg, rays_o, rays_d, particles, rgb, sorted_values, ranges, tile_order, chunk_base, hit_words, out_rgba, out_dist, out_hits, nullptr);
}

void launch_count_work(cudaStream_t s, const FrameCamera& cam, const FrameConfig& cfg, const float* rays_o, const float* rays_d,
                       const float* particles, const float* rgb, const uint32_t* sorted_values, const uint32_t* ranges,
                       const uint32_t* tile_order, const uint32_t* chunk_base, uint32_t* hit_words, unsigned long long* counters8) {
    const unsigned grid = cam.grid_x * cam.grid_y;
    WorkCounters* ctr = reinterpret_cast<WorkCounters*>(counters8);
    if (cfg.kernel_degree == 4)
        render_forward_kernel<4, true><<<grid, kTilePixels, 0, s>>>(cam, cfg, rays_o, rays_d, particles, rgb, sorted_values, ranges, tile_order, chunk_base, hit_words, nullptr, nullptr, nullptr, ctr);
    else
        render_forward_kernel<2, true><<<grid, kTilePixels, 0, s>>>(cam, cfg, rays_o, rays_d, particles, rgb, sorted_values, ranges, tile_order, chunk_base, hit_words, nullptr, nullptr, nullptr, ctr);
}

void launch_render_backward(cudaStream_t s, const FrameCamera& cam, const FrameConfig& cfg, const float* rays_o,
                            const float* rays_d, const float* particles, const float* rgb, const uint32_t* sorted_values,
                            const uint32_t* ranges, const uint32_t* tile_order, const uint32_t* chunk_base, const uint32_t* hit_words,
                            const float* out_rgba, const float* d_rgba, const float* out_dist, const float* d_dist, float* grad_acc) {
    const unsigned grid = cam.grid_x * cam.grid_y;
    const int sub = (cfg.subtile_culling >> 4) & 3;
#define GUT_BWD(DEG_, SUB_) render_backward_kernel<DEG_, SUB_><<<grid, kTilePixels, 0, s>>>(cam, cfg, rays_o, rays_d, particles, rgb, sorted_values, ranges, tile_order, chunk_base, hit_words, out_rgba, d_rgba, out_dist, d_dist, grad_acc)
    if (cfg.kernel_degree == 4) {
        if (sub == 2) GUT_BWD(4, 32); else if (sub == 1) GUT_BWD(4, 16); else GUT_BWD(4, 8);
    } else {
        if (sub == 2) GUT_BWD(2, 32); else if (sub == 1) GUT_BWD(2, 16); else GUT_BWD(2, 8);
    }
#undef GUT_BWD
}

void launch_project_backward(cudaStream_t s, const FrameCamera& cam, int64_t n, const float* particles, const float* sph,
                             int sph_degree, const float* rgb, const uint32_t* tiles_count, const float* rays_o, float* grad_acc,
                             float* d_particles, float* d_sph, bool compact, bool canon, bool radiance) {
    if (n <= 0) return;
    const unsigned blocks = static_cast<unsigned>((n + kPbThreads - 1) / kPbThreads);
    if (!radiance)
        project_backward_kernel<false, true, false><<<blocks, kPbThreads, 0, s>>>(cam, n, particles, nullptr, 0, nullptr, tiles_count, rays_o, grad_acc, d_particles, nullptr);
    else if (compact && canon)
        project_backward_kernel<true, true, true><<<blocks, kPbThreads, 0, s>>>(cam, n, particles, sph, sph_degree, rgb, tiles_count, rays_o, grad_acc, d_particles, d_sph);
    else if (compact)
        project_backward_kernel<true, false, true><<<blocks, kPbThreads, 0, s>>>(cam, n, particles, sph, sph_degree, rgb, tiles_count, rays_o, grad_acc, d_particles, d_sph);
    else if (canon)
        project_backward_kernel<false, true, true><<<blocks, kPbThreads, 0, s>>>(cam, n, particles, sph, sph_degree, rgb, tiles_count, rays_o, grad_acc, d_particles, d_sph);
    else
        project_backward_kernel<false, false, true><<<blocks, kPbThreads, 0, s>>>(cam, n, particles, sph, sph_degree, rgb, tiles_count, rays_o, grad_acc, d_particles, d_sph);
}

void launch_sph_from_views(cudaStream_t s, int64_t n, const float* particles, int sph_degree, int views, const float* view_positions ,
                           const float* d_radiance_all, float* d_sph) {
    if (n <= 0) return;
    ViewPositions vp;
    for (int v = 0; v < views; ++v)
        for (int k = 0; k < 3; ++k) vp.pos[v][k] = view_positions[v * 3 + k];
    const unsigned blocks = static_cast<unsigned>((n + 127) / 128);
    sph_from_views_kernel<<<blocks, 128, 0, s>>>(n, particles, sph_degree, views, vp, reinterpret_cast<const float4*>(d_radiance_all),
                                                 reinterpret_cast<float4*>(d_sph));
}

}
```

### 3dgrut_b200/csrc/gut_render_nht.cu

```cuda
#include <cuda_fp16.h>

#include "gut_common.cuh"
#include "nht_features.cuh"
#include "render_tile.cuh"
#include "subtile_cull.cuh"

namespace gutb200 {

namespace {

constexpr int kNhtBatch = 128;
constexpr int kNhtChannels = kNhtOut + 1;

template <bool HALF>
__device__ __forceinline__ void stage_features(float4 (*feat)[12], const void* __restrict__ features, const uint32_t* __restrict__ sorted_values,
                                               uint32_t base, int count, int tid) {
    if (HALF) {
        const uint4* src = reinterpret_cast<const uint4*>(features);
        for (int f = tid; f < count * 6; f += kTilePixels) {
            const int e = f / 6, part = f - e * 6;
            const uint32_t idx = sorted_values[base + e];
            const uint4 v = __ldg(src + static_cast<size_t>(idx) * 6 + part);
            const float2 a = __half22float2(*reinterpret_cast<const __half2*>(&v.x)), b = __half22float2(*reinterpret_cast<const __half2*>(&v.y));
            const float2 c = __half22float2(*reinterpret_cast<const __half2*>(&v.z)), d = __half22float2(*reinterpret_cast<const __half2*>(&v.w));
            feat[e][part * 2] = make_float4(a.x, a.y, b.x, b.y);
            feat[e][part * 2 + 1] = make_float4(c.x, c.y, d.x, d.y);
        }
    } else {
        const float4* src = reinterpret_cast<const float4*>(features);
        for (int f = tid; f < count * 12; f += kTilePixels) {
            const int e = f / 12, part = f - e * 12;
            const uint32_t idx = sorted_values[base + e];
            feat[e][part] = __ldg(src + static_cast<size_t>(idx) * 12 + part);
        }
    }
}


struct NhtFwdSmem : FwdRecords<kNhtBatch> {
    float4 feat[kNhtBatch][12];
};

template <bool HALF>
struct FeaturePayload {
    float4 (*feat)[12];
    const void* __restrict__ features;
    float acc[kNhtOut];
    __device__ __forceinline__ void entry(int, uint32_t) {}
    __device__ __forceinline__ void batch(const uint32_t* __restrict__ sorted_values, uint32_t base, int count, int tid) {
        stage_features<HALF>(feat, features, sorted_values, base, count, tid);
    }
    __device__ __forceinline__ void add(int j, float w, float px, float py, float pz) {
        float wk[4], b[kNhtBase];
        bary_weights(px, py, pz, wk);
        blend(feat[j], wk, b);
#pragma unroll
        for (int n = 0; n < kNhtBase; ++n) {
            float s, c;
            sincosf(b[n], &s, &c);
            acc[2 * n] += s * w;
            acc[2 * n + 1] += c * w;
        }
    }
};

template <int DEG, bool HALF>
__global__ void __launch_bounds__(kTilePixels) render_forward_nht_kernel(FrameCamera cam, FrameConfig cfg, const float* __restrict__ rays_o,
                                                                         const float* __restrict__ rays_d, const float* __restrict__ particles,
                                                                         const void* __restrict__ features,
                                                                         const uint32_t* __restrict__ sorted_values,
                                                                         const uint32_t* __restrict__ ranges, const uint32_t* __restrict__ tile_order,
                                                                         const uint32_t* __restrict__ chunk_base, uint32_t* __restrict__ hit_words,
                                                                         float* __restrict__ out_features_alpha, float* __restrict__ out_dist,
                                                                         float* __restrict__ out_hits) {
    __shared__ NhtFwdSmem sm;
    const int tid = threadIdx.x;
    const TileRay tr = tile_ray(cam, rays_o, rays_d, tile_order, tid);
    float T = 1.f, dist = 0.f;
    FeaturePayload<HALF> pay{sm.feat, features};
#pragma unroll
    for (int c = 0; c < kNhtOut; ++c) pay.acc[c] = 0.f;
    uint32_t hits = 0;
    forward_list<DEG, false>(cam, cfg, sm, pay, tr, tid, rays_o, particles, sorted_values, ranges, chunk_base, hit_words, T, dist, hits, nullptr);

    const int64_t pix = tr.pix;
    if (!tr.inside) return;
    float* o = out_features_alpha + pix * kNhtChannels;
    if (tr.valid) {
#pragma unroll
        for (int c = 0; c < kNhtOut; ++c) o[c] = pay.acc[c];
        o[kNhtOut] = 1.0f - T;
        out_dist[pix] = dist;
        out_hits[pix] = static_cast<float>(hits);
    } else {
#pragma unroll
        for (int c = 0; c < kNhtChannels; ++c) o[c] = 0.f;
        out_dist[pix] = 1e06f;
        out_hits[pix] = 0.f;
    }
}


struct NhtBwdSmem : BwdRecords<kNhtBatch> {
    float4 feat[kNhtBatch][12];
    uint32_t idx[kNhtBatch];
    uint32_t hw[(kNhtBatch / 32) * kWordsPerChunk];
    float rows[kTilePixels / 32][32][33];
};

struct NhtBwdRay {
    float Tint, Tgrad, Dint, Dgrad, FiG;
    float T, D, FG;
    float g[kNhtOut];
};

struct FeatureHit {
    static constexpr int kDepthSlot = 13;
    static constexpr bool kHitPoint = true;
    float fg;
    __device__ __forceinline__ void at_hit(const NhtBwdSmem& sm, int j, const NhtBwdRay& st, float px, float py, float pz, float weight,
                                           float (&g)[32]) {
        float wk[4], b[kNhtBase];
        bary_weights(px, py, pz, wk);
        blend(sm.feat[j], wk, b);
        fg = 0.f;
#pragma unroll
        for (int n = 0; n < kNhtBase; ++n) {
            float s, c;
            sincosf(b[n], &s, &c);
            fg += s * st.g[2 * n] + c * st.g[2 * n + 1];
            g[20 + n] = weight * (st.g[2 * n] * c - st.g[2 * n + 1] * s);
        }
#pragma unroll
        for (int k = 0; k < 4; ++k) g[16 + k] = wk[k];
    }
    __device__ __forceinline__ float common(const FrameConfig& cfg, NhtBwdRay& st, float T, float weight, float inv_next, float raw_alpha,
                                            float partial, float (&)[32]) {
        st.FG += weight * fg;
        const float res_g = (st.FiG - st.FG) * inv_next;
        float common = partial + T * (fg - res_g);
        if (raw_alpha > cfg.max_alpha) common = 0.f;
        return common;
    }
    __device__ __forceinline__ void hit_point_grad(const NhtBwdSmem& sm, int j, const float (&g)[32], float& pgx, float& pgy, float& pgz) {
        pgx = 0.f; pgy = 0.f; pgz = 0.f;
#pragma unroll
        for (int k = 0; k < 4; ++k) {
            float h = 0.f;
#pragma unroll
            for (int q = 0; q < 3; ++q) {
                const float4 f = sm.feat[j][k * 3 + q];
                h += f.x * g[20 + q * 4] + f.y * g[21 + q * 4] + f.z * g[22 + q * 4] + f.w * g[23 + q * 4];
            }
            pgx += h * kVk12[k][0]; pgy += h * kVk12[k][1]; pgz += h * kVk12[k][2];
        }
    }
};

template <int DEG, bool FAST, bool HALF>
__device__ __forceinline__ void backward_tile_nht(const FrameConfig& cfg, NhtBwdSmem& sm, const Ray& ray, float ofx, float ofy, float ofz, int tid,
                                                  int lane, uint32_t begin, uint32_t end, const float* __restrict__ particles,
                                                  const void* __restrict__ features, const uint32_t* __restrict__ sorted_values,
                                                  const uint32_t* __restrict__ hit_words, bool use_words, bool alive, NhtBwdRay& st,
                                                  float* __restrict__ grad_acc, float* __restrict__ d_features) {
    const float dox = ray.ox - ofx, doy = ray.oy - ofy, doz = ray.oz - ofz;
    const bool depth_grads = __any_sync(kFull, alive && (st.Dgrad != 0.f));
    float (*rows)[33] = sm.rows[tid >> 5];
    const int fk0 = lane / kNhtBase, fn0 = lane - fk0 * kNhtBase;
    const int o1 = lane + 32, fk1 = o1 / kNhtBase, fn1 = o1 - fk1 * kNhtBase;
    const int gslot = lane - 16, gdst = gslot < 13 ? gslot : gslot + 3;
    backward_batches<FAST>(sm, sm.hw, ofx, ofy, ofz, tid, begin, end, particles, sorted_values, hit_words, use_words, alive,
        [&](uint32_t idx) { sm.idx[tid] = idx; },
        [&](uint32_t base, int count) { stage_features<HALF>(sm.feat, features, sorted_values, base, count, tid); },
        [&](int count) {
        for (int c = 0; c < count; c += 32) {
            if (__all_sync(kFull, !alive)) break;
            const uint32_t* hw = sm.hw + (c >> 5) * kWordsPerChunk + (tid >> 5) * 4;
            unsigned todo = hw[0] | hw[1] | hw[2] | hw[3];
            if (count - c < 32) todo &= (1u << (count - c)) - 1u;
            while (todo) {
                const int j = c + __ffs(todo) - 1;
                todo &= todo - 1;
                float g[32];
#pragma unroll
                for (int i = 0; i < 32; ++i) g[i] = 0.f;
                bool hit = false;
                if (alive) hit = backward_pair<DEG, FAST, FeatureHit>(cfg, sm, j, ray, dox, doy, doz, depth_grads, st, alive, g);
                if (__ballot_sync(kFull, hit)) {
#pragma unroll
                    for (int i = 0; i < 32; ++i) rows[lane][i] = g[i];
                    __syncwarp();
                    float f0 = 0.f, f1 = 0.f;
#pragma unroll 8
                    for (int i = 0; i < 32; ++i) {
                        const float* rw = rows[i];
                        f0 += rw[16 + fk0] * rw[20 + fn0];
                        f1 += lane < 16 ? rw[16 + fk1] * rw[20 + fn1] : rw[gslot];
                    }
                    const size_t p = sm.idx[j];
                    if (f0 != 0.f) atomicAdd(d_features + p * kNhtRow + lane, f0);
                    if (f1 != 0.f) {
                        if (lane < 16) atomicAdd(d_features + p * kNhtRow + o1, f1);
                        else atomicAdd(grad_acc + p * kGradRow + gdst, f1);
                    }
                    __syncwarp();
                    if (__all_sync(kFull, !alive)) break;
                }
            }
        }
    });
}

template <int DEG, bool HALF>
__global__ void __launch_bounds__(kTilePixels) render_backward_nht_kernel(FrameCamera cam, FrameConfig cfg, const float* __restrict__ rays_o,
                                                                          const float* __restrict__ rays_d, const float* __restrict__ particles,
                                                                          const void* __restrict__ features,
                                                                          const uint32_t* __restrict__ sorted_values,
                                                                          const uint32_t* __restrict__ ranges, const uint32_t* __restrict__ tile_order,
                                                                          const uint32_t* __restrict__ chunk_base, const uint32_t* __restrict__ hit_words,
                                                                          const float* __restrict__ out_features_alpha,
                                                                          const float* __restrict__ d_features_alpha, const float* __restrict__ out_dist,
                                                                          const float* __restrict__ d_dist, float* __restrict__ grad_acc,
                                                                          float* __restrict__ d_features) {
    extern __shared__ __align__(16) unsigned char smem_raw[];
    NhtBwdSmem& sm = *reinterpret_cast<NhtBwdSmem*>(smem_raw);
    const int tid = threadIdx.x;
    const TileRay tr = tile_ray(cam, rays_o, rays_d, tile_order, tid);
    const int64_t pix = tr.pix;

    NhtBwdRay st;
    st.Tint = 1.f; st.Tgrad = 0.f; st.Dint = 0.f; st.Dgrad = 0.f; st.FiG = 0.f;
    st.T = 1.f; st.D = 0.f; st.FG = 0.f;
#pragma unroll
    for (int c = 0; c < kNhtOut; ++c) st.g[c] = 0.f;
    if (tr.valid) {
        const float* o = out_features_alpha + pix * kNhtChannels;
        const float* d = d_features_alpha + pix * kNhtChannels;
#pragma unroll
        for (int c = 0; c < kNhtOut; ++c) {
            st.g[c] = d[c];
            st.FiG += o[c] * st.g[c];
        }
        st.Tint = 1.f - o[kNhtOut];
        st.Tgrad = -1.f * d[kNhtOut];
        st.Dint = out_dist[pix];
        st.Dgrad = d_dist[pix];
    }

    float ofx, ofy, ofz;
    const bool fast = frame_common_origin(cam, rays_o, tr.inside, pix, ofx, ofy, ofz);
    const uint32_t begin = ranges[tr.tile * 2], end = ranges[tr.tile * 2 + 1];
    const uint32_t* words = hit_words + static_cast<size_t>(chunk_base[tr.tile]) * kWordsPerChunk;
    const bool use_words = (cfg.subtile_culling & 4) != 0;
    if (fast)
        backward_tile_nht<DEG, true, HALF>(cfg, sm, tr.ray, ofx, ofy, ofz, tid, tid & 31, begin, end, particles, features, sorted_values, words, use_words, tr.valid, st, grad_acc, d_features);
    else
        backward_tile_nht<DEG, false, HALF>(cfg, sm, tr.ray, ofx, ofy, ofz, tid, tid & 31, begin, end, particles, features, sorted_values, words, use_words, tr.valid, st, grad_acc, d_features);
}

}

void launch_render_forward_nht(cudaStream_t s, const FrameCamera& cam, const FrameConfig& cfg, const float* rays_o, const float* rays_d,
                               const float* particles, const void* features, bool half, const uint32_t* sorted_values, const uint32_t* ranges,
                               const uint32_t* tile_order, const uint32_t* chunk_base, uint32_t* hit_words, float* out_features_alpha,
                               float* out_dist, float* out_hits) {
    const unsigned grid = cam.grid_x * cam.grid_y;
#define GUT_NHT_FWD(DEG_, HALF_) render_forward_nht_kernel<DEG_, HALF_><<<grid, kTilePixels, 0, s>>>(cam, cfg, rays_o, rays_d, particles, features, sorted_values, ranges, tile_order, chunk_base, hit_words, out_features_alpha, out_dist, out_hits)
    if (cfg.kernel_degree == 4) {
        if (half) GUT_NHT_FWD(4, true); else GUT_NHT_FWD(4, false);
    } else {
        if (half) GUT_NHT_FWD(2, true); else GUT_NHT_FWD(2, false);
    }
#undef GUT_NHT_FWD
}

cudaError_t launch_render_backward_nht(cudaStream_t s, const FrameCamera& cam, const FrameConfig& cfg, const float* rays_o, const float* rays_d,
                                       const float* particles, const void* features, bool half, const uint32_t* sorted_values,
                                       const uint32_t* ranges, const uint32_t* tile_order, const uint32_t* chunk_base, const uint32_t* hit_words,
                                       const float* out_features_alpha, const float* d_features_alpha, const float* out_dist, const float* d_dist,
                                       float* grad_acc, float* d_features) {
    const unsigned grid = cam.grid_x * cam.grid_y;
    const int bytes = static_cast<int>(sizeof(NhtBwdSmem));
    cudaError_t e = cudaSuccess;
#define GUT_NHT_BWD(DEG_, HALF_)                                                                                                          \
    do {                                                                                                                                  \
        e = cudaFuncSetAttribute(render_backward_nht_kernel<DEG_, HALF_>, cudaFuncAttributeMaxDynamicSharedMemorySize, bytes);          \
        if (e != cudaSuccess) return e;                                                                                                   \
        render_backward_nht_kernel<DEG_, HALF_><<<grid, kTilePixels, bytes, s>>>(cam, cfg, rays_o, rays_d, particles, features, sorted_values, \
                                                                                  ranges, tile_order, chunk_base, hit_words, out_features_alpha, \
                                                                                  d_features_alpha, out_dist, d_dist, grad_acc, d_features);   \
    } while (0)
    if (cfg.kernel_degree == 4) {
        if (half) GUT_NHT_BWD(4, true); else GUT_NHT_BWD(4, false);
    } else {
        if (half) GUT_NHT_BWD(2, true); else GUT_NHT_BWD(2, false);
    }
#undef GUT_NHT_BWD
    return cudaGetLastError();
}

}
```

### 3dgrut_b200/csrc/render_tile.cuh

```cuda
#pragma once
#include "gut_common.cuh"
#include "subtile_cull.cuh"

namespace gutb200 {

namespace {

constexpr unsigned kFull = 0xFFFFFFFFu;
struct Ray {
    float ox, oy, oz, dx, dy, dz, tmin, tmax;
    bool alive;
};

__device__ __forceinline__ Ray make_ray(const FrameCamera& cam, const float* __restrict__ rays_o, const float* __restrict__ rays_d,
                                        int64_t pix) {
    Ray r;
    const float rox = rays_o[pix * 3 + 0], roy = rays_o[pix * 3 + 1], roz = rays_o[pix * 3 + 2];
    const float rdx = rays_d[pix * 3 + 0], rdy = rays_d[pix * 3 + 1], rdz = rays_d[pix * 3 + 2];
    const float* m = cam.s2w;
    r.ox = m[0] * rox + m[3] * roy + m[6] * roz + m[9];
    r.oy = m[1] * rox + m[4] * roy + m[7] * roz + m[10];
    r.oz = m[2] * rox + m[5] * roy + m[8] * roz + m[11];
    r.dx = m[0] * rdx + m[3] * rdy + m[6] * rdz;
    r.dy = m[1] * rdx + m[4] * rdy + m[7] * rdz;
    r.dz = m[2] * rdx + m[5] * rdy + m[8] * rdz;
    const float lo = -1e06f, hi = 1e06f;
    float tmin = (lo - r.ox) / r.dx, tmax = (hi - r.ox) / r.dx, t;
    if (tmin > tmax) { t = tmin; tmin = tmax; tmax = t; }
    float tymin = (lo - r.oy) / r.dy, tymax = (hi - r.oy) / r.dy;
    if (tymin > tymax) { t = tymin; tymin = tymax; tymax = t; }
    bool miss = (tmin > tymax) || (tymin > tmax);
    tmin = fmaxf(tmin, tymin);
    tmax = fminf(tmax, tymax);
    float tzmin = (lo - r.oz) / r.dz, tzmax = (hi - r.oz) / r.dz;
    if (tzmin > tzmax) { t = tzmin; tzmin = tzmax; tzmax = t; }
    miss = miss || (tmin > tzmax) || (tzmin > tmax);
    tmin = fmaxf(tmin, tzmin);
    tmax = fminf(tmax, tzmax);
    r.tmin = miss ? 3.4028235e+38f : fmaxf(tmin, 0.0f);
    r.tmax = miss ? 3.4028235e+38f : tmax;
    r.alive = r.tmax > r.tmin;
    return r;
}

template <int DEG>
__device__ __forceinline__ float kernel_response(float gray) {
    if (DEG == 4) return __expf(-0.0555555555556f * gray * gray);
    return __expf(-0.5f * gray);
}

template <int DEG>
__device__ __forceinline__ float kernel_response_grad(float gray, float gres, float gres_grad) {
    if (DEG == 4) return (-0.0555555555556f * 2.0f) * gray * gres * gres_grad;
    return -0.5f * gres * gres_grad;
}

__device__ __forceinline__ WarpFrame make_warp_frame(const FrameCamera& cam, const Ray& ray, bool alive, bool enabled, int lane) {
    WarpFrame wf;
    wf.on = false;
    const unsigned live = __ballot_sync(kFull, alive);
    if (!enabled || live == 0u) return wf;
    const int src = __ffs(live) - 1;
    float dx = __shfl_sync(kFull, ray.dx, src), dy = __shfl_sync(kFull, ray.dy, src), dz = __shfl_sync(kFull, ray.dz, src);
    if (!frame_axes(cam.s2w, dx, dy, dz, wf)) return wf;
    float u = 0.f, v = 0.f;
    const bool fine = !alive || ray_uv(wf, ray.dx, ray.dy, ray.dz, u, v);
    float ulo = alive ? u : 3.0e38f, uhi = alive ? u : -3.0e38f, vlo = alive ? v : 3.0e38f, vhi = alive ? v : -3.0e38f;
#pragma unroll
    for (int o = 16; o > 0; o >>= 1) {
        ulo = fminf(ulo, __shfl_xor_sync(kFull, ulo, o));
        uhi = fmaxf(uhi, __shfl_xor_sync(kFull, uhi, o));
        vlo = fminf(vlo, __shfl_xor_sync(kFull, vlo, o));
        vhi = fmaxf(vhi, __shfl_xor_sync(kFull, vhi, o));
    }
    wf.ulo = ulo; wf.uhi = uhi; wf.vlo = vlo; wf.vhi = vhi;
    wf.umax = fmaxf(fmaxf(fabsf(ulo), fabsf(uhi)), fmaxf(fabsf(vlo), fabsf(vhi)));
    wf.on = __all_sync(kFull, fine);
    return wf;
}

__device__ __forceinline__ void tile_pixel(int tile, int grid_x, int tid, int& px, int& py) {
    const int tx = tile % grid_x, ty = tile / grid_x;
    px = tx * kTile + ((tid >> 5) & 1) * 8 + (tid & 7);
    py = ty * kTile + (tid >> 6) * 4 + ((tid >> 3) & 3);
}

__device__ __forceinline__ bool tile_common_origin(const FrameCamera& cam, const float* __restrict__ rays_o, int tile, bool inside,
                                                   int64_t pix, float& ox, float& oy, float& oz) {
    const int tx = tile % cam.grid_x, ty = tile / cam.grid_x;
    const int64_t pix0 = static_cast<int64_t>(ty * kTile) * cam.width + tx * kTile;
    const float ax = rays_o[pix0 * 3 + 0], ay = rays_o[pix0 * 3 + 1], az = rays_o[pix0 * 3 + 2];
    bool same = true;
    if (inside) same = (rays_o[pix * 3 + 0] == ax) && (rays_o[pix * 3 + 1] == ay) && (rays_o[pix * 3 + 2] == az);
    const float* m = cam.s2w;
    ox = m[0] * ax + m[3] * ay + m[6] * az + m[9];
    oy = m[1] * ax + m[4] * ay + m[7] * az + m[10];
    oz = m[2] * ax + m[5] * ay + m[8] * az + m[11];
    return __syncthreads_and(same);
}

__device__ __forceinline__ int lane_quarter(int lane) { return ((lane >> 2) & 1) | ((lane >> 3) & 2); }
__device__ __forceinline__ unsigned quarter_lanes(int q) { return (0x0F0Fu << ((q & 1) * 4)) << ((q >> 1) * 16); }
constexpr int kWordsPerChunk = (kTilePixels / 32) * 4;
__device__ __forceinline__ bool frame_common_origin(const FrameCamera& cam, const float* __restrict__ rays_o, bool inside, int64_t pix,
                                                    float& ox, float& oy, float& oz) {
    const float ax = rays_o[0], ay = rays_o[1], az = rays_o[2];
    bool same = true;
    if (inside) same = (rays_o[pix * 3 + 0] == ax) && (rays_o[pix * 3 + 1] == ay) && (rays_o[pix * 3 + 2] == az);
    const float* m = cam.s2w;
    ox = m[0] * ax + m[3] * ay + m[6] * az + m[9];
    oy = m[1] * ax + m[4] * ay + m[7] * az + m[10];
    oz = m[2] * ax + m[5] * ay + m[8] * az + m[11];
    return __syncthreads_and(same);
}

struct TileRay {
    int tile;
    bool inside, valid;
    int64_t pix;
    Ray ray;
};

__device__ __forceinline__ TileRay tile_ray(const FrameCamera& cam, const float* __restrict__ rays_o, const float* __restrict__ rays_d,
                                            const uint32_t* __restrict__ tile_order, int tid) {
    TileRay t;
    t.tile = tile_order[blockIdx.x];
    int px, py;
    tile_pixel(t.tile, cam.grid_x, tid, px, py);
    t.inside = (px < cam.width) && (py < cam.height);
    t.pix = static_cast<int64_t>(py) * cam.width + px;
    t.ray.alive = false;
    if (t.inside) t.ray = make_ray(cam, rays_o, rays_d, t.pix);
    t.valid = t.inside && t.ray.alive;
    return t;
}

__device__ __forceinline__ void rotation_rows(const float4& q, float3& r0, float3& r1, float3& r2) {
    const float r = q.x, x = q.y, y = q.z, z = q.w;
    const float xx = x * x, yy = y * y, zz = z * z, xy = x * y, xz = x * z, yz = y * z;
    const float rx = r * x, ry = r * y, rz = r * z;
    r0 = make_float3(1.f - 2.f * (yy + zz), 2.f * (xy + rz), 2.f * (xz - ry));
    r1 = make_float3(2.f * (xy - rz), 1.f - 2.f * (xx + zz), 2.f * (yz + rx));
    r2 = make_float3(2.f * (xz + ry), 2.f * (yz - rx), 1.f - 2.f * (xx + yy));
}


template <int B>
struct FwdRecords {
    float4 m0[B], m1[B], m2[B], sd[B];
};

template <bool UNIFORM, int B>
__device__ __forceinline__ void stage_fwd_record(FwdRecords<B>& sm, int slot, const float* __restrict__ particles, uint32_t idx, float o0x,
                                                 float o0y, float o0z) {
    const float4* p4 = reinterpret_cast<const float4*>(particles) + static_cast<size_t>(idx) * 3;
    const float4 a = __ldg(p4), q = __ldg(p4 + 1), s = __ldg(p4 + 2);
    float3 r0, r1, r2;
    rotation_rows(q, r0, r1, r2);
    const float isx = 1.0f / s.x, isy = 1.0f / s.y, isz = 1.0f / s.z;
    float4 m0 = make_float4(isx * r0.x, isx * r0.y, isx * r0.z, a.x);
    float4 m1 = make_float4(isy * r1.x, isy * r1.y, isy * r1.z, a.y);
    float4 m2 = make_float4(isz * r2.x, isz * r2.y, isz * r2.z, a.z);
    if (UNIFORM) {
        const float vx = o0x - a.x, vy = o0y - a.y, vz = o0z - a.z;
        m0.w = m0.x * vx + m0.y * vy + m0.z * vz;
        m1.w = m1.x * vx + m1.y * vy + m1.z * vz;
        m2.w = m2.x * vx + m2.y * vy + m2.z * vz;
    }
    sm.m0[slot] = m0;
    sm.m1[slot] = m1;
    sm.m2[slot] = m2;
    sm.sd[slot] = make_float4(s.x, s.y, s.z, a.w);
}

template <int DEG, bool UNIFORM, int B, class Payload>
__device__ __forceinline__ bool forward_pair(const FrameConfig& cfg, const FwdRecords<B>& sm, Payload& pay, int j, const Ray& ray, bool& alive,
                                             float& T, float& dist, uint32_t& hits) {
    const float4 m0 = sm.m0[j], m1 = sm.m1[j], m2 = sm.m2[j];
    float gox, goy, goz;
    if (UNIFORM) {
        gox = m0.w; goy = m1.w; goz = m2.w;
    } else {
        const float vx = ray.ox - m0.w, vy = ray.oy - m1.w, vz = ray.oz - m2.w;
        gox = m0.x * vx + m0.y * vy + m0.z * vz;
        goy = m1.x * vx + m1.y * vy + m1.z * vz;
        goz = m2.x * vx + m2.y * vy + m2.z * vz;
    }
    const float ax = m0.x * ray.dx + m0.y * ray.dy + m0.z * ray.dz;
    const float ay = m1.x * ray.dx + m1.y * ray.dy + m1.z * ray.dz;
    const float az = m2.x * ray.dx + m2.y * ray.dy + m2.z * ray.dz;
    const float l = ax * ax + ay * ay + az * az;
    const float il = l > 0.f ? rsqrtf(l) : 1.f;
    const float gdx = ax * il, gdy = ay * il, gdz = az * il;
    const float ccx = gdy * goz - gdz * goy, ccy = gdz * gox - gdx * goz, ccz = gdx * goy - gdy * gox;
    const float gray = ccx * ccx + ccy * ccy + ccz * ccz;
    const float gres = kernel_response<DEG>(gray);
    const float4 sd = sm.sd[j];
    const float alpha = fminf(cfg.max_alpha, gres * sd.w);
    const bool accept = (gres > cfg.min_kernel_density) && (alpha > cfg.min_alpha);
    if (accept) {
        const float pd = -(gdx * gox + gdy * goy + gdz * goz);
        const float hx = sd.x * gdx * pd, hy = sd.y * gdy * pd, hz = sd.z * gdz * pd;
        const float t = sqrtf(hx * hx + hy * hy + hz * hz);
        if ((t > ray.tmin) && (t < ray.tmax)) {
            const float w = alpha * T;
            dist += t * w;
            T *= (1.f - alpha);
            if (w > 0.f) {
                pay.add(j, w, gox + gdx * pd, goy + gdy * pd, goz + gdz * pd);
                hits++;
            }
            if (T < cfg.min_transmittance) alive = false;
        }
    }
    return accept;
}

struct WorkCounters {
    unsigned long long v[16];
};

template <int DEG, bool UNIFORM, bool COUNT, int B, class Payload>
__device__ __forceinline__ void forward_tile(const FrameConfig& cfg, FwdRecords<B>& sm, Payload& pay, const WarpFrame& wf, const Ray& ray, float o0x,
                                             float o0y, float o0z, int tid, uint32_t begin, uint32_t end, const float* __restrict__ particles,
                                             const uint32_t* __restrict__ sorted_values, uint32_t* __restrict__ hit_words, bool& alive, float& T,
                                             float& dist, uint32_t& hits, WorkCounters* __restrict__ ctr) {
    const int lane = tid & 31;
    unsigned long long c_ref = 0, c_exec = 0, c_hits = 0, c_iters = 0, c_hit_iters = 0, c_screens = 0, c_bwd_lanes = 0;
    unsigned long long c_iters16 = 0, c_iters8 = 0, c_sub16 = 0, c_sub8 = 0;
    for (uint32_t base = begin; base < end; base += B) {
        if (__syncthreads_and(!alive)) break;
        const int count = min(B, static_cast<int>(end - base));
        const uint32_t k = base + tid;
        if ((B >= kTilePixels || tid < B) && k < end) {
            const uint32_t idx = sorted_values[k];
            stage_fwd_record<UNIFORM>(sm, tid, particles, idx, o0x, o0y, o0z);
            pay.entry(tid, idx);
        }
        pay.batch(sorted_values, base, count, tid);
        __syncthreads();
        uint32_t* words = hit_words + (static_cast<size_t>(base - begin) >> 5) * kWordsPerChunk + (tid >> 5) * 4;
        const int quarter = lane_quarter(lane);
        const unsigned my_quarter = quarter_lanes(quarter);
        const bool writer = (lane & 0x0B) == 0;
        if (UNIFORM) {
            for (int c = 0; c < count; c += 32) {
                if (!__any_sync(kFull, alive)) break;
                const int e = c + lane;
                bool cand = e < count;
                if (wf.on && cand) {
                    const float4 m0 = sm.m0[e], m1 = sm.m1[e], m2 = sm.m2[e];
                    cand = block_candidate<DEG>(cfg, wf, m0.x, m0.y, m0.z, m1.x, m1.y, m1.z, m2.x, m2.y, m2.z, m0.w, m1.w, m2.w, sm.sd[e].w);
                    if (COUNT) c_screens++;
                }
                unsigned todo = __ballot_sync(kFull, cand);
                uint32_t word = 0;
                int prev = c;
                while (todo) {
                    const int b = __ffs(todo) - 1;
                    const int j = c + b;
                    todo &= todo - 1;
                    int live_n = 0;
                    if (COUNT) {
                        live_n = __popc(__ballot_sync(kFull, alive));
                        c_ref += static_cast<unsigned long long>(live_n) * (j - prev + 1);
                        prev = j + 1;
                        c_iters++;
                        if (alive) c_exec++;
                    }
                    bool acc = false;
                    if (alive) acc = forward_pair<DEG, true>(cfg, sm, pay, j, ray, alive, T, dist, hits);
                    const unsigned accs = __ballot_sync(kFull, acc);
                    if (accs & my_quarter) word |= 1u << b;
                    if (COUNT && accs) {
                        c_hit_iters++;
                        c_bwd_lanes += live_n;
                        c_hits += acc ? 1 : 0;
                    }
                }
                if (COUNT) {
                    const unsigned live = __ballot_sync(kFull, alive);
                    c_ref += static_cast<unsigned long long>(__popc(live)) * (min(c + 32, count) - prev);
                    const uint32_t wq = word, wh = word | __shfl_xor_sync(kFull, word, 16);
                    const int p16 = __popc(wh), p8 = __popc(wq);
                    const int m16 = max(p16, __shfl_xor_sync(kFull, p16, 4));
                    int m8 = max(p8, __shfl_xor_sync(kFull, p8, 4));
                    m8 = max(m8, __shfl_xor_sync(kFull, m8, 16));
                    c_iters16 += m16;
                    c_iters8 += m8;
                    c_sub16 += p16 + __shfl_xor_sync(kFull, p16, 4);
                    int s8 = p8 + __shfl_xor_sync(kFull, p8, 4);
                    s8 += __shfl_xor_sync(kFull, s8, 16);
                    c_sub8 += s8;
                }
                if (writer) words[(c >> 5) * kWordsPerChunk + quarter] = word;
            }
        } else {
            if (writer)
                for (int c = 0; c < count; c += 32) words[(c >> 5) * kWordsPerChunk + quarter] = 0xFFFFFFFFu;
            for (int j = 0; alive && j < count; ++j) {
                const bool acc = forward_pair<DEG, false>(cfg, sm, pay, j, ray, alive, T, dist, hits);
                if (COUNT) {
                    c_exec++;
                    c_hits += acc ? 1 : 0;
                }
            }
        }
    }
    if (COUNT) {
        if (!UNIFORM) c_ref = 0;
#pragma unroll
        for (int o = 16; o > 0; o >>= 1) {
            c_exec += __shfl_xor_sync(kFull, c_exec, o);
            c_hits += __shfl_xor_sync(kFull, c_hits, o);
            c_screens += __shfl_xor_sync(kFull, c_screens, o);
        }
        if (lane == 0) {
            if (!UNIFORM) c_ref = c_exec;
            atomicAdd(&ctr->v[0], c_ref);
            atomicAdd(&ctr->v[1], c_exec);
            atomicAdd(&ctr->v[2], c_hits);
            atomicAdd(&ctr->v[3], c_iters);
            atomicAdd(&ctr->v[4], c_hit_iters);
            atomicAdd(&ctr->v[5], c_screens);
            atomicAdd(&ctr->v[6], c_bwd_lanes);
            atomicAdd(&ctr->v[7], c_iters16);
            atomicAdd(&ctr->v[8], c_iters8);
            atomicAdd(&ctr->v[9], c_sub16);
            atomicAdd(&ctr->v[10], c_sub8);
        }
    }
}

template <int DEG, bool COUNT, int B, class Payload>
__device__ __forceinline__ void forward_list(const FrameCamera& cam, const FrameConfig& cfg, FwdRecords<B>& sm, Payload& pay, const TileRay& tr,
                                             int tid, const float* __restrict__ rays_o, const float* __restrict__ particles,
                                             const uint32_t* __restrict__ sorted_values, const uint32_t* __restrict__ ranges,
                                             const uint32_t* __restrict__ chunk_base, uint32_t* __restrict__ hit_words, float& T, float& dist,
                                             uint32_t& hits, WorkCounters* __restrict__ ctr) {
    float o0x, o0y, o0z;
    const bool uniform = tile_common_origin(cam, rays_o, tr.tile, tr.inside, tr.pix, o0x, o0y, o0z);
    const WarpFrame wf = make_warp_frame(cam, tr.ray, tr.valid, uniform && (cfg.subtile_culling & 2), tid & 31);
    bool alive = tr.valid;
    const uint32_t begin = ranges[tr.tile * 2], end = ranges[tr.tile * 2 + 1];
    uint32_t* words = hit_words + static_cast<size_t>(chunk_base[tr.tile]) * kWordsPerChunk;
    if (uniform)
        forward_tile<DEG, true, COUNT>(cfg, sm, pay, wf, tr.ray, o0x, o0y, o0z, tid, begin, end, particles, sorted_values, words, alive, T, dist, hits, ctr);
    else
        forward_tile<DEG, false, COUNT>(cfg, sm, pay, wf, tr.ray, o0x, o0y, o0z, tid, begin, end, particles, sorted_values, words, alive, T, dist, hits, ctr);
}


template <int B>
struct BwdRecords {
    float4 r0[B], r1[B], r2[B], sc[B], is[B];
};

template <bool FAST, int B>
__device__ __forceinline__ void stage_bwd_record(BwdRecords<B>& sm, int slot, const float* __restrict__ particles, uint32_t idx, float ofx,
                                                 float ofy, float ofz) {
    const float4* p4 = reinterpret_cast<const float4*>(particles) + static_cast<size_t>(idx) * 3;
    const float4 a = __ldg(p4), q = __ldg(p4 + 1), s = __ldg(p4 + 2);
    float3 r0, r1, r2;
    rotation_rows(q, r0, r1, r2);
    float4 t0 = make_float4(r0.x, r0.y, r0.z, a.x);
    float4 t1 = make_float4(r1.x, r1.y, r1.z, a.y);
    float4 t2 = make_float4(r2.x, r2.y, r2.z, a.z);
    if (FAST) {
        const float vx = ofx - a.x, vy = ofy - a.y, vz = ofz - a.z;
        t0.w = (t0.x * vx + t0.y * vy + t0.z * vz) / s.x;
        t1.w = (t1.x * vx + t1.y * vy + t1.z * vz) / s.y;
        t2.w = (t2.x * vx + t2.y * vy + t2.z * vz) / s.z;
    }
    sm.r0[slot] = t0;
    sm.r1[slot] = t1;
    sm.r2[slot] = t2;
    sm.sc[slot] = make_float4(s.x, s.y, s.z, a.w);
    sm.is[slot] = make_float4(1.0f / s.x, 1.0f / s.y, 1.0f / s.z, 0.f);
}

template <bool FAST, int B, class Entry, class Batch, class Walk>
__device__ __forceinline__ void backward_batches(BwdRecords<B>& sm, uint32_t* hw, float ofx, float ofy, float ofz, int tid, uint32_t begin,
                                                 uint32_t end, const float* __restrict__ particles, const uint32_t* __restrict__ sorted_values,
                                                 const uint32_t* __restrict__ hit_words, bool use_words, const bool& alive, Entry&& entry,
                                                 Batch&& batch, Walk&& walk) {
    constexpr int kWords = (B / 32) * kWordsPerChunk;
    for (uint32_t base = begin; base < end; base += B) {
        if (__syncthreads_and(!alive)) break;
        const int count = min(B, static_cast<int>(end - base));
        if (kWords >= kTilePixels || tid < kWords) {
            const uint32_t chunk = (base - begin) / 32 + (tid >> 5);
            const bool in_list = base + (tid >> 5) * 32 < end;
            hw[tid] = (use_words && in_list) ? hit_words[static_cast<size_t>(chunk) * kWordsPerChunk + (tid & 31)] : 0xFFFFFFFFu;
        }
        const uint32_t k = base + tid;
        if ((B >= kTilePixels || tid < B) && k < end) {
            const uint32_t idx = sorted_values[k];
            stage_bwd_record<FAST>(sm, tid, particles, idx, ofx, ofy, ofz);
            entry(idx);
        }
        batch(base, count);
        __syncthreads();
        walk(count);
    }
}

template <int DEG, bool FAST, class Kind, class Smem, class St, int NG>
__device__ __forceinline__ bool backward_pair(const FrameConfig& cfg, const Smem& sm, int j, const Ray& ray, float dox, float doy, float doz,
                                              bool depth_grads, St& st, bool& alive, float (&g)[NG]) {
    const float4 r0 = sm.r0[j], r1 = sm.r1[j], r2 = sm.r2[j], sc = sm.sc[j], is = sm.is[j];
    float gox, goy, goz;
    if (FAST) {
        gox = r0.w; goy = r1.w; goz = r2.w;
    } else {
        const float pcx = ray.ox - r0.w, pcy = ray.oy - r1.w, pcz = ray.oz - r2.w;
        gox = is.x * (r0.x * pcx + r0.y * pcy + r0.z * pcz);
        goy = is.y * (r1.x * pcx + r1.y * pcy + r1.z * pcz);
        goz = is.z * (r2.x * pcx + r2.y * pcy + r2.z * pcz);
    }
    const float drx = r0.x * ray.dx + r0.y * ray.dy + r0.z * ray.dz;
    const float dry = r1.x * ray.dx + r1.y * ray.dy + r1.z * ray.dz;
    const float drz = r2.x * ray.dx + r2.y * ray.dy + r2.z * ray.dz;
    const float ux = is.x * drx, uy = is.y * dry, uz = is.z * drz;
    const float l = ux * ux + uy * uy + uz * uz;
    const float il = l > 0.f ? rsqrtf(l) : 1.f;
    const float gdx = ux * il, gdy = uy * il, gdz = uz * il;
    const float ccx = gdy * goz - gdz * goy, ccy = gdz * gox - gdx * goz, ccz = gdx * goy - gdy * gox;
    const float gray = ccx * ccx + ccy * ccy + ccz * ccz;
    const float gres = kernel_response<DEG>(gray);
    const float dns = sc.w;
    const float raw_alpha = gres * dns;
    const float alpha = fminf(cfg.max_alpha, raw_alpha);
    if (!((gres > cfg.min_kernel_density) && (alpha > cfg.min_alpha))) return false;

    const float T = st.T;
    const float weight = alpha * T;
    const float nextT = (1.f - alpha) * T;
    const bool last = nextT <= cfg.min_transmittance;
    const float inv_next = last ? 0.f : 1.0f / nextT;
    const float pd = -(gdx * gox + gdy * goy + gdz * goz);
    Kind kind;
    kind.at_hit(sm, j, st, gox + gdx * pd, goy + gdy * pd, goz + gdz * pd, weight, g);

    float a_hit = 0.f, sd = 0.f, hgx = 0.f, hgy = 0.f, hgz = 0.f, ddx = 0.f, ddy = 0.f, ddz = 0.f;
    if (depth_grads) {
        ddx = gdx * pd; ddy = gdy * pd; ddz = gdz * pd;
        const float hx = sc.x * ddx, hy = sc.y * ddy, hz = sc.z * ddz;
        const float gsq = hx * hx + hy * hy + hz * hz;
        const float gdist = sqrtf(gsq);
        st.D += weight * gdist;
        const float resD = fmaxf((st.Dint - st.D) * inv_next, 0.f);
        a_hit = (gdist - resD) * T * st.Dgrad;
        const float hs = gsq > 0.f ? (weight / gdist) * st.Dgrad : 0.f;
        hgx = hx * hs; hgy = hy * hs; hgz = hz * hs;
        sd = hgx * sc.x * gdx + hgy * sc.y * gdy + hgz * sc.z * gdz;
    }
    const float resT = alpha < 0.999999f ? st.Tint / (1.f - alpha) : T;
    const float a_dns = resT * -st.Tgrad;
    const float common = kind.common(cfg, st, T, weight, inv_next, raw_alpha, a_hit + a_dns, g);
    g[3] = gres * common;
    const float gray_g = kernel_response_grad<DEG>(gray, gres, dns * common);
    const float kx = 2.f * ccx * gray_g, ky = 2.f * ccy * gray_g, kz = 2.f * ccz * gray_g;
    float go_gx = ky * gdz - kz * gdy, go_gy = kz * gdx - kx * gdz, go_gz = kx * gdy - ky * gdx;
    float ug_x, ug_y, ug_z;
    if (depth_grads) {
        const float sd2 = 2.f * sd;
        const float vx = (go_gx + sc.x * hgx) - sd2 * gdx, vy = (go_gy + sc.y * hgy) - sd2 * gdy, vz = (go_gz + sc.z * hgz) - sd2 * gdz;
        ug_x = il * (pd * vx - sd * gox); ug_y = il * (pd * vy - sd * goy); ug_z = il * (pd * vz - sd * goz);
        go_gx -= gdx * sd; go_gy -= gdy * sd; go_gz -= gdz * sd;
        constexpr int D = Kind::kDepthSlot;
        g[D] = ddx * hgx; g[D + 1] = ddy * hgy; g[D + 2] = ddz * hgz;
    } else {
        const float tq = pd * il;
        ug_x = tq * go_gx; ug_y = tq * go_gy; ug_z = tq * go_gz;
    }
    if constexpr (Kind::kHitPoint) {
        float pgx, pgy, pgz;
        kind.hit_point_grad(sm, j, g, pgx, pgy, pgz);
        const float s = gdx * pgx + gdy * pgy + gdz * pgz;
        go_gx += pgx - gdx * s; go_gy += pgy - gdy * s; go_gz += pgz - gdz * s;
        const float ps2 = 2.f * pd * s;
        ug_x += il * (pd * pgx - s * gox - ps2 * gdx);
        ug_y += il * (pd * pgy - s * goy - ps2 * gdy);
        ug_z += il * (pd * pgz - s * goz - ps2 * gdz);
    }
    g[0] = go_gx; g[1] = go_gy; g[2] = go_gz;
    g[4] = ug_x * ray.dx; g[5] = ug_x * ray.dy; g[6] = ug_x * ray.dz;
    g[7] = ug_y * ray.dx; g[8] = ug_y * ray.dy; g[9] = ug_y * ray.dz;
    g[10] = ug_z * ray.dx; g[11] = ug_z * ray.dy; g[12] = ug_z * ray.dz;
    if (!FAST) {
        g[4] += go_gx * dox; g[5] += go_gx * doy; g[6] += go_gx * doz;
        g[7] += go_gy * dox; g[8] += go_gy * doy; g[9] += go_gy * doz;
        g[10] += go_gz * dox; g[11] += go_gz * doy; g[12] += go_gz * doz;
    }
    st.T = nextT;
    if (nextT < cfg.min_transmittance) alive = false;
    return true;
}

}

}
```

Before: 1056.

## Fuse small-tile depth sort into forward render kernel and drop hit-word memset

After: 1069, median of 6. 1.01x the previous value.

```diff
diff --git a/3dgrut_b200/csrc/gut_api.cu b/3dgrut_b200/csrc/gut_api.cu
--- a/3dgrut_b200/csrc/gut_api.cu
+++ b/3dgrut_b200/csrc/gut_api.cu
@@ -438,23 +438,24 @@
             {
                 StageTimer t(c, 3, s);
                 GUT_CUDA(c, launch_tile_sort(s, static_cast<int>(tiles), c->tile_order.as<uint32_t>(), c->ranges.as<uint32_t>(), c->totals.as<uint32_t>(),
-                                             c->keys64.as<unsigned long long>(), c->keys64_alt.as<unsigned long long>(), c->vals_out.as<uint32_t>()));
+                                             c->keys64.as<unsigned long long>(), c->keys64_alt.as<unsigned long long>(), c->vals_out.as<uint32_t>(),
+                                             c->fcfg.k_buffer_size == 0 ? kFwdSliceKeys : 0u));
             }
             c->launches += 2;
         }
         {
             StageTimer t(c, 5, s);
-            if (c->fcfg.k_buffer_size == 0)
-                GUT_CUDA(c, cudaMemsetAsync(c->hit_words.ptr, 0, hit_words_capacity(capacity, tiles) * 4, s));
             if (nht)
-                launch_render_forward_nht(s, c->cam, c->fcfg, rays_o, rays_d, particles, sph, half, c->vals_out.as<uint32_t>(),
+                launch_render_forward_nht(s, c->cam, c->fcfg, rays_o, rays_d, particles, sph, half, c->keys64.as<unsigned long long>(),
+                                          c->vals_out.as<uint32_t>(),
                                           c->ranges.as<uint32_t>(), c->tile_order.as<uint32_t>(), c->chunk_base.as<uint32_t>(),
                                           c->hit_words.as<uint32_t>(), out_rgba, out_dist, out_hits);
             else if (c->fcfg.k_buffer_size > 0)
                 launch_render_forward_kbuffer(s, c->cam, c->fcfg, c->fcfg.k_buffer_size, rays_o, rays_d, particles, c->rgb.as<float>(),
                                               c->vals_out.as<uint32_t>(), c->ranges.as<uint32_t>(), out_rgba, out_dist, out_hits);
             else
-                launch_render_forward(s, c->cam, c->fcfg, rays_o, rays_d, particles, c->rgb.as<float>(), c->vals_out.as<uint32_t>(),
+                launch_render_forward(s, c->cam, c->fcfg, rays_o, rays_d, particles, c->rgb.as<float>(), c->keys64.as<unsigned long long>(),
+                                      c->vals_out.as<uint32_t>(),
                                       c->ranges.as<uint32_t>(), c->tile_order.as<uint32_t>(), c->chunk_base.as<uint32_t>(),
                                       c->hit_words.as<uint32_t>(), out_rgba, out_dist, out_hits);
         }
diff --git a/3dgrut_b200/csrc/gut_binning.cu b/3dgrut_b200/csrc/gut_binning.cu
--- a/3dgrut_b200/csrc/gut_binning.cu
+++ b/3dgrut_b200/csrc/gut_binning.cu
@@ -1,6 +1,7 @@
 #include <cstdlib>
 
 #include "gut_common.cuh"
+#include "tile_sort.cuh"
 
 namespace gutb200 {
 
@@ -140,135 +141,37 @@
 }
 
 
-
-constexpr int kSortThreads = 512, kSortWarps = kSortThreads / 32;
+constexpr int kSortThreads = 512;
 constexpr int kSortUnroll = 4;
-constexpr int kStageKeys = 4096, kStagePerLane = kStageKeys / kSortThreads;
-
-__device__ __forceinline__ bool scan_digits(uint32_t (*s_cnt)[256], uint32_t* s_tot, int* s_flag, int aw, uint32_t n) {
-    const int lane = threadIdx.x & 31, warp = threadIdx.x >> 5, d = threadIdx.x;
-    uint32_t tot = 0, incl = 0;
-    if (d < 256) {
-        for (int w = 0; w < aw; ++w) tot += s_cnt[w][d];
-        if (tot == n) *s_flag = 1;
-        incl = tot;
-#pragma unroll
-        for (int o = 1; o < 32; o <<= 1) {
-            const uint32_t v = __shfl_up_sync(kFullMask, incl, o);
-            if (lane >= o) incl += v;
-        }
-        if (lane == 31) s_tot[warp] = incl;
-    }
-    __syncthreads();
-    const bool skip = *s_flag != 0;
-    if (!skip && d < 256) {
-        uint32_t run = incl - tot;
-        for (int w = 0; w < warp; ++w) run += s_tot[w];
-        for (int w = 0; w < aw; ++w) {
-            const uint32_t c = s_cnt[w][d];
-            s_cnt[w][d] = run;
-            run += c;
-        }
-    }
-    __syncthreads();
-    return skip;
-}
-
-template <bool BALLOT>
-__device__ __forceinline__ uint32_t rank_key(uint32_t* cnt_row, unsigned long long k, int shift, bool have) {
-    const int lane = threadIdx.x & 31;
-    const uint32_t dg = have ? (static_cast<uint32_t>(k >> shift) & 255u) : 256u + lane;
-    unsigned peers;
-    if (BALLOT) {
-        peers = __ballot_sync(kFullMask, have);
-#pragma unroll
-        for (int b = 0; b < 8; ++b) {
-            const bool bit = (dg >> b) & 1u;
-            const unsigned bal = __ballot_sync(kFullMask, bit);
-            peers &= bit ? bal : ~bal;
-        }
-        if (!have) peers = 1u << lane;
-    } else {
-        peers = __match_any_sync(kFullMask, dg);
-    }
-    const int leader = __ffs(peers) - 1;
-    uint32_t slot = 0;
-    if (have && lane == leader) slot = atomicAdd(&cnt_row[dg], static_cast<uint32_t>(__popc(peers)));
-    slot = __shfl_sync(kFullMask, slot, leader);
-    return slot + __popc(peers & ((1u << lane) - 1u));
-}
-
-__device__ __forceinline__ void fix_equal_depth_runs(unsigned long long* a, uint32_t n) {
-    for (uint32_t i = threadIdx.x; i + 1 < n; i += kSortThreads) {
-        const unsigned long long x = a[i];
-        if ((x >> 32) != (a[i + 1] >> 32)) continue;
-        if (i > 0 && (a[i - 1] >> 32) == (x >> 32)) continue;
-        uint32_t e = i + 2;
-        while (e < n && (a[e] >> 32) == (x >> 32)) ++e;
-        for (uint32_t p = i + 1; p < e; ++p) {
-            const unsigned long long k = a[p];
-            uint32_t q = p;
-            while (q > i && a[q - 1] > k) {
-                a[q] = a[q - 1];
-                --q;
-            }
-            a[q] = k;
-        }
-    }
-}
 
 template <bool BALLOT>
 __global__ void __launch_bounds__(kSortThreads) tile_sort_kernel(const uint32_t* __restrict__ order, const uint32_t* __restrict__ ranges,
                                                                  const uint32_t* __restrict__ totals, unsigned long long* keys,
-                                                                 unsigned long long* keys_alt, uint32_t* __restrict__ sorted_values) {
-    __shared__ uint32_t s_cnt[kSortWarps][256];
-    __shared__ uint32_t s_tot[8];
-    __shared__ int s_flag;
+                                                                 unsigned long long* keys_alt, uint32_t* __restrict__ sorted_values,
+                                                                 uint32_t forward_sorts) {
+    __shared__ SliceSortSmem<kSortThreads> ss;
     extern __shared__ unsigned long long s_keys[];
     if (totals[1] != 0u) return;
     const uint32_t tile = order[blockIdx.x];
     const uint32_t begin = ranges[tile * 2], n = ranges[tile * 2 + 1] - begin;
     if (n == 0u) return;
-    const int lane = threadIdx.x & 31, warp = threadIdx.x >> 5;
     unsigned long long* src = keys + begin;
     unsigned long long* dst = keys_alt + begin;
-    const int aw = static_cast<int>(min(static_cast<uint32_t>(kSortWarps), max(1u, (n + 127u) / 128u)));
+
+    if (n <= static_cast<uint32_t>(kSliceKeys)) {
+        if (n <= forward_sorts) return;
+        sort_slice<kSortThreads, kSliceKeys, BALLOT>(src, s_keys, ss, n);
+        for (uint32_t i = threadIdx.x; i < n; i += kSortThreads) sorted_values[begin + i] = static_cast<uint32_t>(s_keys[i]);
+        return;
+    }
+
+    const int lane = threadIdx.x & 31, warp = threadIdx.x >> 5;
+    const int aw = sort_warps<kSortThreads>(n);
     const uint32_t seg = ((n + aw - 1) / aw + 31u) & ~31u;
     const uint32_t w0 = min(n, warp * seg), w1 = min(n, w0 + seg);
-
-    if (n <= static_cast<uint32_t>(kStageKeys)) {
-        for (uint32_t i = threadIdx.x; i < n; i += kSortThreads) s_keys[i] = src[i];
-        for (int shift = 32; shift < 64; shift += 8) {
-            for (int i = threadIdx.x; i < aw * 256; i += kSortThreads) (&s_cnt[0][0])[i] = 0u;
-            if (threadIdx.x == 0) s_flag = 0;
-            __syncthreads();
-            unsigned long long k[kStagePerLane];
-#pragma unroll
-            for (int u = 0; u < kStagePerLane; ++u) {
-                const uint32_t i = w0 + u * 32 + lane;
-                k[u] = i < w1 ? s_keys[i] : 0ull;
-                if (i < w1) atomicAdd(&s_cnt[warp][static_cast<uint32_t>(k[u] >> shift) & 255u], 1u);
-            }
-            __syncthreads();
-            if (scan_digits(s_cnt, s_tot, &s_flag, aw, n)) continue;
-#pragma unroll
-            for (int u = 0; u < kStagePerLane; ++u) {
-                if (w0 + u * 32 >= w1) break;
-                const bool have = w0 + u * 32 + lane < w1;
-                const uint32_t slot = rank_key<BALLOT>(s_cnt[warp], k[u], shift, have);
-                if (have) s_keys[slot] = k[u];
-            }
-            __syncthreads();
-        }
-        fix_equal_depth_runs(s_keys, n);
-        __syncthreads();
-        for (uint32_t i = threadIdx.x; i < n; i += kSortThreads) sorted_values[begin + i] = static_cast<uint32_t>(s_keys[i]);
-        return;
-    }
-
     for (int shift = 32; shift < 64; shift += 8) {
-        for (int i = threadIdx.x; i < aw * 256; i += kSortThreads) (&s_cnt[0][0])[i] = 0u;
-        if (threadIdx.x == 0) s_flag = 0;
+        for (int i = threadIdx.x; i < aw * 256; i += kSortThreads) (&ss.cnt[0][0])[i] = 0u;
+        if (threadIdx.x == 0) ss.flag = 0;
         __syncthreads();
         for (uint32_t i0 = w0; i0 < w1; i0 += 32 * kSortUnroll) {
             unsigned long long k[kSortUnroll];
@@ -279,10 +182,10 @@
             }
 #pragma unroll
             for (int u = 0; u < kSortUnroll; ++u)
-                if (i0 + u * 32 + lane < w1) atomicAdd(&s_cnt[warp][static_cast<uint32_t>(k[u] >> shift) & 255u], 1u);
+                if (i0 + u * 32 + lane < w1) atomicAdd(&ss.cnt[warp][static_cast<uint32_t>(k[u] >> shift) & 255u], 1u);
         }
         __syncthreads();
-        if (scan_digits(s_cnt, s_tot, &s_flag, aw, n)) continue;
+        if (scan_digits(ss.cnt, ss.tot, &ss.flag, aw, n)) continue;
         for (uint32_t i0 = w0; i0 < w1; i0 += 32 * kSortUnroll) {
             unsigned long long k[kSortUnroll];
 #pragma unroll
@@ -294,7 +197,7 @@
             for (int u = 0; u < kSortUnroll; ++u) {
                 if (i0 + u * 32 >= w1) break;
                 const bool have = i0 + u * 32 + lane < w1;
-                const uint32_t slot = rank_key<BALLOT>(s_cnt[warp], k[u], shift, have);
+                const uint32_t slot = rank_key<BALLOT>(ss.cnt[warp], k[u], shift, have);
                 if (have) dst[slot] = k[u];
             }
         }
@@ -303,7 +206,7 @@
         src = dst;
         dst = t;
     }
-    fix_equal_depth_runs(src, n);
+    fix_equal_depth_runs<kSortThreads>(src, n);
     __syncthreads();
     for (uint32_t i = threadIdx.x; i < n; i += kSortThreads) sorted_values[begin + i] = static_cast<uint32_t>(src[i]);
 }
@@ -328,10 +231,10 @@
 }
 
 cudaError_t launch_tile_sort(cudaStream_t s, int num_tiles, const uint32_t* order, const uint32_t* ranges, const uint32_t* totals,
-                             unsigned long long* keys, unsigned long long* keys_alt, uint32_t* sorted_values) {
+                             unsigned long long* keys, unsigned long long* keys_alt, uint32_t* sorted_values, uint32_t forward_sorts) {
     if (num_tiles <= 0) return cudaSuccess;
     static const bool use_match = [] { const char* e = std::getenv("GUTB200_SORT_MATCH"); return e && std::atoi(e) != 0; }();
-    constexpr size_t kStageBytes = kStageKeys * sizeof(unsigned long long);
+    constexpr size_t kStageBytes = kSliceKeys * sizeof(unsigned long long);
     static const cudaError_t opt_in = [] {
         cudaError_t e = cudaFuncSetAttribute(tile_sort_kernel<false>, cudaFuncAttributeMaxDynamicSharedMemorySize, static_cast<int>(kStageBytes));
         if (e == cudaSuccess)
@@ -340,9 +243,9 @@
     }();
     if (opt_in != cudaSuccess) return opt_in;
     if (use_match)
-        tile_sort_kernel<false><<<num_tiles, kSortThreads, kStageBytes, s>>>(order, ranges, totals, keys, keys_alt, sorted_values);
+        tile_sort_kernel<false><<<num_tiles, kSortThreads, kStageBytes, s>>>(order, ranges, totals, keys, keys_alt, sorted_values, forward_sorts);
     else
-        tile_sort_kernel<true><<<num_tiles, kSortThreads, kStageBytes, s>>>(order, ranges, totals, keys, keys_alt, sorted_values);
+        tile_sort_kernel<true><<<num_tiles, kSortThreads, kStageBytes, s>>>(order, ranges, totals, keys, keys_alt, sorted_values, forward_sorts);
     return cudaGetLastError();
 }
 
diff --git a/3dgrut_b200/csrc/gut_common.cuh b/3dgrut_b200/csrc/gut_common.cuh
--- a/3dgrut_b200/csrc/gut_common.cuh
+++ b/3dgrut_b200/csrc/gut_common.cuh
@@ -56,13 +56,14 @@
 size_t tile_scan_parts_words(int num_tiles);
 void launch_tile_scan(cudaStream_t s, int num_tiles, const uint32_t* counts, uint32_t capacity, uint32_t* ranges, uint32_t* sub_base,
                       uint32_t* chunk_base, uint32_t* order, uint32_t* fill, uint32_t* totals, uint32_t* parts);
+constexpr int kFwdSliceKeys = 2048;
 cudaError_t launch_tile_sort(cudaStream_t s, int num_tiles, const uint32_t* order, const uint32_t* ranges, const uint32_t* totals,
-                             unsigned long long* keys, unsigned long long* keys_alt, uint32_t* sorted_values);
+                             unsigned long long* keys, unsigned long long* keys_alt, uint32_t* sorted_values, uint32_t forward_sorts);
 void launch_synth_tile_keys(cudaStream_t s, int num_tiles, const uint32_t* ranges, const uint32_t* vals, const float* depth, uint64_t* out);
 
 inline size_t hit_words_capacity(int64_t num_isect, int64_t tiles) { return (static_cast<size_t>(num_isect) / 32 + static_cast<size_t>(tiles) + 1) * 32; }
 void launch_render_forward(cudaStream_t s, const FrameCamera& cam, const FrameConfig& cfg, const float* rays_o,
-                           const float* rays_d, const float* particles, const float* rgb, const uint32_t* sorted_values,
+                           const float* rays_d, const float* particles, const float* rgb, const unsigned long long* keys, uint32_t* sorted_values,
                            const uint32_t* ranges, const uint32_t* tile_order, const uint32_t* chunk_base, uint32_t* hit_words, float* out_rgba,
                            float* out_dist, float* out_hits);
 void launch_count_work(cudaStream_t s, const FrameCamera& cam, const FrameConfig& cfg, const float* rays_o, const float* rays_d,
@@ -73,8 +74,8 @@
                             const uint32_t* ranges, const uint32_t* tile_order, const uint32_t* chunk_base, const uint32_t* hit_words,
                             const float* out_rgba, const float* d_rgba, const float* out_dist, const float* d_dist, float* grad_acc);
 void launch_render_forward_nht(cudaStream_t s, const FrameCamera& cam, const FrameConfig& cfg, const float* rays_o, const float* rays_d,
-                               const float* particles, const void* features, bool half, const uint32_t* sorted_values, const uint32_t* ranges,
-                               const uint32_t* tile_order, const uint32_t* chunk_base, uint32_t* hit_words, float* out_features_alpha,
+                               const float* particles, const void* features, bool half, const unsigned long long* keys, uint32_t* sorted_values,
+                               const uint32_t* ranges, const uint32_t* tile_order, const uint32_t* chunk_base, uint32_t* hit_words, float* out_features_alpha,
                                float* out_dist, float* out_hits);
 cudaError_t launch_render_backward_nht(cudaStream_t s, const FrameCamera& cam, const FrameConfig& cfg, const float* rays_o, const float* rays_d,
                                        const float* particles, const void* features, bool half, const uint32_t* sorted_values,
diff --git a/3dgrut_b200/csrc/gut_render.cu b/3dgrut_b200/csrc/gut_render.cu
--- a/3dgrut_b200/csrc/gut_render.cu
+++ b/3dgrut_b200/csrc/gut_render.cu
@@ -38,19 +38,21 @@
                                                                      const float* __restrict__ rays_d,
                                                                      const float* __restrict__ particles,
                                                                      const float* __restrict__ rgb,
-                                                                     const uint32_t* __restrict__ sorted_values,
+                                                                     const unsigned long long* __restrict__ keys,
+                                                                     uint32_t* __restrict__ sorted_values,
                                                                      const uint32_t* __restrict__ ranges,
                                                                      const uint32_t* __restrict__ tile_order,
                                                                      const uint32_t* __restrict__ chunk_base, uint32_t* __restrict__ hit_words,
                                                                      float* __restrict__ out_rgba, float* __restrict__ out_dist,
                                                                      float* __restrict__ out_hits, WorkCounters* __restrict__ ctr) {
-    __shared__ FwdSmem sm;
+    __shared__ FwdTileSmem<FwdSmem> sm;
     const int tid = threadIdx.x;
+    const TileList tl = forward_sort<!COUNT>(sm, tile_order, ranges, keys, sorted_values, tid);
     const TileRay tr = tile_ray(cam, rays_o, rays_d, tile_order, tid);
-    RadiancePayload pay{sm.col, rgb};
+    RadiancePayload pay{sm.w.walk.col, rgb};
     float T = 1.f, dist = 0.f;
     uint32_t hits = 0;
-    forward_list<DEG, COUNT>(cam, cfg, sm, pay, tr, tid, rays_o, particles, sorted_values, ranges, chunk_base, hit_words, T, dist, hits, ctr);
+    forward_list<DEG, COUNT>(cam, cfg, sm, pay, tr, tl, tid, rays_o, particles, chunk_base, hit_words, T, dist, hits, ctr);
     if (COUNT) return;
 
     const int64_t pix = tr.pix;
@@ -433,14 +435,14 @@
 }
 
 void launch_render_forward(cudaStream_t s, const FrameCamera& cam, const FrameConfig& cfg, const float* rays_o,
-                           const float* rays_d, const float* particles, const float* rgb, const uint32_t* sorted_values,
+                           const float* rays_d, const float* particles, const float* rgb, const unsigned long long* keys, uint32_t* sorted_values,
                            const uint32_t* ranges, const uint32_t* tile_order, const uint32_t* chunk_base, uint32_t* hit_words, float* out_rgba,
                            float* out_dist, float* out_hits) {
     const unsigned grid = cam.grid_x * cam.grid_y;
     if (cfg.kernel_degree == 4)
-        render_forward_kernel<4, false><<<grid, kTilePixels, 0, s>>>(cam, cfg, rays_o, rays_d, particles, rgb, sorted_values, ranges, tile_order, chunk_base, hit_words, out_rgba, out_dist, out_hits, nullptr);
+        render_forward_kernel<4, false><<<grid, kTilePixels, 0, s>>>(cam, cfg, rays_o, rays_d, particles, rgb, keys, sorted_values, ranges, tile_order, chunk_base, hit_words, out_rgba, out_dist, out_hits, nullptr);
     else
-        render_forward_kernel<2, false><<<grid, kTilePixels, 0, s>>>(cam, cfg, rays_o, rays_d, particles, rgb, sorted_values, ranges, tile_order, chunk_base, hit_words, out_rgba, out_dist, out_hits, nullptr);
+        render_forward_kernel<2, false><<<grid, kTilePixels, 0, s>>>(cam, cfg, rays_o, rays_d, particles, rgb, keys, sorted_values, ranges, tile_order, chunk_base, hit_words, out_rgba, out_dist, out_hits, nullptr);
 }
 
 void launch_count_work(cudaStream_t s, const FrameCamera& cam, const FrameConfig& cfg, const float* rays_o, const float* rays_d,
@@ -448,10 +450,11 @@
                        const uint32_t* tile_order, const uint32_t* chunk_base, uint32_t* hit_words, unsigned long long* counters8) {
     const unsigned grid = cam.grid_x * cam.grid_y;
     WorkCounters* ctr = reinterpret_cast<WorkCounters*>(counters8);
+    uint32_t* vals = const_cast<uint32_t*>(sorted_values);
     if (cfg.kernel_degree == 4)
-        render_forward_kernel<4, true><<<grid, kTilePixels, 0, s>>>(cam, cfg, rays_o, rays_d, particles, rgb, sorted_values, ranges, tile_order, chunk_base, hit_words, nullptr, nullptr, nullptr, ctr);
+        render_forward_kernel<4, true><<<grid, kTilePixels, 0, s>>>(cam, cfg, rays_o, rays_d, particles, rgb, nullptr, vals, ranges, tile_order, chunk_base, hit_words, nullptr, nullptr, nullptr, ctr);
     else
-        render_forward_kernel<2, true><<<grid, kTilePixels, 0, s>>>(cam, cfg, rays_o, rays_d, particles, rgb, sorted_values, ranges, tile_order, chunk_base, hit_words, nullptr, nullptr, nullptr, ctr);
+        render_forward_kernel<2, true><<<grid, kTilePixels, 0, s>>>(cam, cfg, rays_o, rays_d, particles, rgb, nullptr, vals, ranges, tile_order, chunk_base, hit_words, nullptr, nullptr, nullptr, ctr);
 }
 
 void launch_render_backward(cudaStream_t s, const FrameCamera& cam, const FrameConfig& cfg, const float* rays_o,
diff --git a/3dgrut_b200/csrc/gut_render_nht.cu b/3dgrut_b200/csrc/gut_render_nht.cu
--- a/3dgrut_b200/csrc/gut_render_nht.cu
+++ b/3dgrut_b200/csrc/gut_render_nht.cu
@@ -13,7 +13,7 @@
 constexpr int kNhtChannels = kNhtOut + 1;
 
 template <bool HALF>
-__device__ __forceinline__ void stage_features(float4 (*feat)[12], const void* __restrict__ features, const uint32_t* __restrict__ sorted_values,
+__device__ __forceinline__ void stage_features(float4 (*feat)[12], const void* __restrict__ features, const uint32_t* sorted_values,
                                                uint32_t base, int count, int tid) {
     if (HALF) {
         const uint4* src = reinterpret_cast<const uint4*>(features);
@@ -47,8 +47,8 @@
     const void* __restrict__ features;
     float acc[kNhtOut];
     __device__ __forceinline__ void entry(int, uint32_t) {}
-    __device__ __forceinline__ void batch(const uint32_t* __restrict__ sorted_values, uint32_t base, int count, int tid) {
-        stage_features<HALF>(feat, features, sorted_values, base, count, tid);
+    __device__ __forceinline__ void batch(const uint32_t* vals, uint32_t base, int count, int tid) {
+        stage_features<HALF>(feat, features, vals, base, count, tid);
     }
     __device__ __forceinline__ void add(int j, float w, float px, float py, float pz) {
         float wk[4], b[kNhtBase];
@@ -68,20 +68,22 @@
 __global__ void __launch_bounds__(kTilePixels) render_forward_nht_kernel(FrameCamera cam, FrameConfig cfg, const float* __restrict__ rays_o,
                                                                          const float* __restrict__ rays_d, const float* __restrict__ particles,
                                                                          const void* __restrict__ features,
-                                                                         const uint32_t* __restrict__ sorted_values,
+                                                                         const unsigned long long* __restrict__ keys,
+                                                                         uint32_t* __restrict__ sorted_values,
                                                                          const uint32_t* __restrict__ ranges, const uint32_t* __restrict__ tile_order,
                                                                          const uint32_t* __restrict__ chunk_base, uint32_t* __restrict__ hit_words,
                                                                          float* __restrict__ out_features_alpha, float* __restrict__ out_dist,
                                                                          float* __restrict__ out_hits) {
-    __shared__ NhtFwdSmem sm;
+    __shared__ FwdTileSmem<NhtFwdSmem> sm;
     const int tid = threadIdx.x;
+    const TileList tl = forward_sort<true>(sm, tile_order, ranges, keys, sorted_values, tid);
     const TileRay tr = tile_ray(cam, rays_o, rays_d, tile_order, tid);
     float T = 1.f, dist = 0.f;
-    FeaturePayload<HALF> pay{sm.feat, features};
+    FeaturePayload<HALF> pay{sm.w.walk.feat, features};
 #pragma unroll
     for (int c = 0; c < kNhtOut; ++c) pay.acc[c] = 0.f;
     uint32_t hits = 0;
-    forward_list<DEG, false>(cam, cfg, sm, pay, tr, tid, rays_o, particles, sorted_values, ranges, chunk_base, hit_words, T, dist, hits, nullptr);
+    forward_list<DEG, false>(cam, cfg, sm, pay, tr, tl, tid, rays_o, particles, chunk_base, hit_words, T, dist, hits, nullptr);
 
     const int64_t pix = tr.pix;
     if (!tr.inside) return;
@@ -261,11 +263,11 @@
 }
 
 void launch_render_forward_nht(cudaStream_t s, const FrameCamera& cam, const FrameConfig& cfg, const float* rays_o, const float* rays_d,
-                               const float* particles, const void* features, bool half, const uint32_t* sorted_values, const uint32_t* ranges,
-                               const uint32_t* tile_order, const uint32_t* chunk_base, uint32_t* hit_words, float* out_features_alpha,
+                               const float* particles, const void* features, bool half, const unsigned long long* keys, uint32_t* sorted_values,
+                               const uint32_t* ranges, const uint32_t* tile_order, const uint32_t* chunk_base, uint32_t* hit_words, float* out_features_alpha,
                                float* out_dist, float* out_hits) {
     const unsigned grid = cam.grid_x * cam.grid_y;
-#define GUT_NHT_FWD(DEG_, HALF_) render_forward_nht_kernel<DEG_, HALF_><<<grid, kTilePixels, 0, s>>>(cam, cfg, rays_o, rays_d, particles, features, sorted_values, ranges, tile_order, chunk_base, hit_words, out_features_alpha, out_dist, out_hits)
+#define GUT_NHT_FWD(DEG_, HALF_) render_forward_nht_kernel<DEG_, HALF_><<<grid, kTilePixels, 0, s>>>(cam, cfg, rays_o, rays_d, particles, features, keys, sorted_values, ranges, tile_order, chunk_base, hit_words, out_features_alpha, out_dist, out_hits)
     if (cfg.kernel_degree == 4) {
         if (half) GUT_NHT_FWD(4, true); else GUT_NHT_FWD(4, false);
     } else {
diff --git a/3dgrut_b200/csrc/render_tile.cuh b/3dgrut_b200/csrc/render_tile.cuh
--- a/3dgrut_b200/csrc/render_tile.cuh
+++ b/3dgrut_b200/csrc/render_tile.cuh
@@ -1,6 +1,7 @@
 #pragma once
 #include "gut_common.cuh"
 #include "subtile_cull.cuh"
+#include "tile_sort.cuh"
 
 namespace gutb200 {
 
@@ -150,6 +151,18 @@
     float4 m0[B], m1[B], m2[B], sd[B];
 };
 
+template <class Walk>
+union FwdTileSmem {
+    struct {
+        unsigned long long keys[kFwdSliceKeys];
+        SliceSortSmem<kTilePixels> sort;
+    } s;
+    struct {
+        uint32_t idx[kFwdSliceKeys];
+        Walk walk;
+    } w;
+};
+
 template <bool UNIFORM, int B>
 __device__ __forceinline__ void stage_fwd_record(FwdRecords<B>& sm, int slot, const float* __restrict__ particles, uint32_t idx, float o0x,
                                                  float o0y, float o0z) {
@@ -223,21 +236,26 @@
 template <int DEG, bool UNIFORM, bool COUNT, int B, class Payload>
 __device__ __forceinline__ void forward_tile(const FrameConfig& cfg, FwdRecords<B>& sm, Payload& pay, const WarpFrame& wf, const Ray& ray, float o0x,
                                              float o0y, float o0z, int tid, uint32_t begin, uint32_t end, const float* __restrict__ particles,
-                                             const uint32_t* __restrict__ sorted_values, uint32_t* __restrict__ hit_words, bool& alive, float& T,
-                                             float& dist, uint32_t& hits, WorkCounters* __restrict__ ctr) {
+                                             const uint32_t* vals, uint32_t* __restrict__ hit_words, bool& alive, float& T, float& dist,
+                                             uint32_t& hits, WorkCounters* __restrict__ ctr) {
     const int lane = tid & 31;
     unsigned long long c_ref = 0, c_exec = 0, c_hits = 0, c_iters = 0, c_hit_iters = 0, c_screens = 0, c_bwd_lanes = 0;
     unsigned long long c_iters16 = 0, c_iters8 = 0, c_sub16 = 0, c_sub8 = 0;
     for (uint32_t base = begin; base < end; base += B) {
-        if (__syncthreads_and(!alive)) break;
+        if (__syncthreads_and(!alive)) {
+            if ((lane & 0x0B) == 0)
+                for (uint32_t c = base - begin; c < end - begin; c += 32)
+                    hit_words[static_cast<size_t>(c >> 5) * kWordsPerChunk + (tid >> 5) * 4 + lane_quarter(lane)] = 0u;
+            break;
+        }
         const int count = min(B, static_cast<int>(end - base));
         const uint32_t k = base + tid;
         if ((B >= kTilePixels || tid < B) && k < end) {
-            const uint32_t idx = sorted_values[k];
+            const uint32_t idx = vals[k - begin];
             stage_fwd_record<UNIFORM>(sm, tid, particles, idx, o0x, o0y, o0z);
             pay.entry(tid, idx);
         }
-        pay.batch(sorted_values, base, count, tid);
+        pay.batch(vals, base - begin, count, tid);
         __syncthreads();
         uint32_t* words = hit_words + (static_cast<size_t>(base - begin) >> 5) * kWordsPerChunk + (tid >> 5) * 4;
         const int quarter = lane_quarter(lane);
@@ -245,7 +263,11 @@
         const bool writer = (lane & 0x0B) == 0;
         if (UNIFORM) {
             for (int c = 0; c < count; c += 32) {
-                if (!__any_sync(kFull, alive)) break;
+                if (!__any_sync(kFull, alive)) {
+                    if (writer)
+                        for (int z = c; z < count; z += 32) words[(z >> 5) * kWordsPerChunk + quarter] = 0u;
+                    break;
+                }
                 const int e = c + lane;
                 bool cand = e < count;
                 if (wf.on && cand) {
@@ -332,22 +354,50 @@
     }
 }
 
-template <int DEG, bool COUNT, int B, class Payload>
-__device__ __forceinline__ void forward_list(const FrameCamera& cam, const FrameConfig& cfg, FwdRecords<B>& sm, Payload& pay, const TileRay& tr,
-                                             int tid, const float* __restrict__ rays_o, const float* __restrict__ particles,
-                                             const uint32_t* __restrict__ sorted_values, const uint32_t* __restrict__ ranges,
+struct TileList {
+    uint32_t begin, end;
+    const uint32_t* vals;
+};
+
+template <bool SORT, class Walk>
+__device__ __forceinline__ TileList forward_sort(FwdTileSmem<Walk>& sm, const uint32_t* __restrict__ tile_order, const uint32_t* __restrict__ ranges,
+                                                 const unsigned long long* __restrict__ keys, uint32_t* __restrict__ sorted_values, int tid) {
+    const uint32_t tile = tile_order[blockIdx.x];
+    TileList tl;
+    tl.begin = ranges[tile * 2];
+    tl.end = ranges[tile * 2 + 1];
+    tl.vals = sorted_values + tl.begin;
+    const uint32_t n = tl.end - tl.begin;
+    if (SORT && n > 0u && n <= static_cast<uint32_t>(kFwdSliceKeys)) {
+        sort_slice<kTilePixels, kFwdSliceKeys, true>(keys + tl.begin, sm.s.keys, sm.s.sort, n);
+        for (uint32_t i0 = 0; i0 < n; i0 += kTilePixels) {
+            const uint32_t i = i0 + tid;
+            const uint32_t v = i < n ? static_cast<uint32_t>(sm.s.keys[i]) : 0u;
+            __syncthreads();
+            if (i < n) {
+                sm.w.idx[i] = v;
+                sorted_values[tl.begin + i] = v;
+            }
+        }
+        tl.vals = sm.w.idx;
+    }
+    return tl;
+}
+
+template <int DEG, bool COUNT, class Walk, class Payload>
+__device__ __forceinline__ void forward_list(const FrameCamera& cam, const FrameConfig& cfg, FwdTileSmem<Walk>& sm, Payload& pay, const TileRay& tr,
+                                             const TileList& tl, int tid, const float* __restrict__ rays_o, const float* __restrict__ particles,
                                              const uint32_t* __restrict__ chunk_base, uint32_t* __restrict__ hit_words, float& T, float& dist,
                                              uint32_t& hits, WorkCounters* __restrict__ ctr) {
     float o0x, o0y, o0z;
     const bool uniform = tile_common_origin(cam, rays_o, tr.tile, tr.inside, tr.pix, o0x, o0y, o0z);
     const WarpFrame wf = make_warp_frame(cam, tr.ray, tr.valid, uniform && (cfg.subtile_culling & 2), tid & 31);
     bool alive = tr.valid;
-    const uint32_t begin = ranges[tr.tile * 2], end = ranges[tr.tile * 2 + 1];
     uint32_t* words = hit_words + static_cast<size_t>(chunk_base[tr.tile]) * kWordsPerChunk;
     if (uniform)
-        forward_tile<DEG, true, COUNT>(cfg, sm, pay, wf, tr.ray, o0x, o0y, o0z, tid, begin, end, particles, sorted_values, words, alive, T, dist, hits, ctr);
+        forward_tile<DEG, true, COUNT>(cfg, sm.w.walk, pay, wf, tr.ray, o0x, o0y, o0z, tid, tl.begin, tl.end, particles, tl.vals, words, alive, T, dist, hits, ctr);
     else
-        forward_tile<DEG, false, COUNT>(cfg, sm, pay, wf, tr.ray, o0x, o0y, o0z, tid, begin, end, particles, sorted_values, words, alive, T, dist, hits, ctr);
+        forward_tile<DEG, false, COUNT>(cfg, sm.w.walk, pay, wf, tr.ray, o0x, o0y, o0z, tid, tl.begin, tl.end, particles, tl.vals, words, alive, T, dist, hits, ctr);
 }
 
 
diff --git a/3dgrut_b200/csrc/tile_sort.cuh b/3dgrut_b200/csrc/tile_sort.cuh
--- /dev/null
+++ b/3dgrut_b200/csrc/tile_sort.cuh
@@ -0,0 +1,134 @@
+#pragma once
+#include "gut_common.cuh"
+
+namespace gutb200 {
+
+namespace {
+
+constexpr unsigned kSortMask = 0xFFFFFFFFu;
+constexpr int kSliceKeys = 4096;
+
+template <int THREADS>
+struct SliceSortSmem {
+    uint32_t cnt[THREADS / 32][256];
+    uint32_t tot[8];
+    int flag;
+};
+
+__device__ __forceinline__ bool scan_digits(uint32_t (*s_cnt)[256], uint32_t* s_tot, int* s_flag, int aw, uint32_t n) {
+    const int lane = threadIdx.x & 31, warp = threadIdx.x >> 5, d = threadIdx.x;
+    uint32_t tot = 0, incl = 0;
+    if (d < 256) {
+        for (int w = 0; w < aw; ++w) tot += s_cnt[w][d];
+        if (tot == n) *s_flag = 1;
+        incl = tot;
+#pragma unroll
+        for (int o = 1; o < 32; o <<= 1) {
+            const uint32_t v = __shfl_up_sync(kSortMask, incl, o);
+            if (lane >= o) incl += v;
+        }
+        if (lane == 31) s_tot[warp] = incl;
+    }
+    __syncthreads();
+    const bool skip = *s_flag != 0;
+    if (!skip && d < 256) {
+        uint32_t run = incl - tot;
+        for (int w = 0; w < warp; ++w) run += s_tot[w];
+        for (int w = 0; w < aw; ++w) {
+            const uint32_t c = s_cnt[w][d];
+            s_cnt[w][d] = run;
+            run += c;
+        }
+    }
+    __syncthreads();
+    return skip;
+}
+
+template <bool BALLOT>
+__device__ __forceinline__ uint32_t rank_key(uint32_t* cnt_row, unsigned long long k, int shift, bool have) {
+    const int lane = threadIdx.x & 31;
+    const uint32_t dg = have ? (static_cast<uint32_t>(k >> shift) & 255u) : 256u + lane;
+    unsigned peers;
+    if (BALLOT) {
+        peers = __ballot_sync(kSortMask, have);
+#pragma unroll
+        for (int b = 0; b < 8; ++b) {
+            const bool bit = (dg >> b) & 1u;
+            const unsigned bal = __ballot_sync(kSortMask, bit);
+            peers &= bit ? bal : ~bal;
+        }
+        if (!have) peers = 1u << lane;
+    } else {
+        peers = __match_any_sync(kSortMask, dg);
+    }
+    const int leader = __ffs(peers) - 1;
+    uint32_t slot = 0;
+    if (have && lane == leader) slot = atomicAdd(&cnt_row[dg], static_cast<uint32_t>(__popc(peers)));
+    slot = __shfl_sync(kSortMask, slot, leader);
+    return slot + __popc(peers & ((1u << lane) - 1u));
+}
+
+template <int THREADS>
+__device__ __forceinline__ void fix_equal_depth_runs(unsigned long long* a, uint32_t n) {
+    for (uint32_t i = threadIdx.x; i + 1 < n; i += THREADS) {
+        const unsigned long long x = a[i];
+        if ((x >> 32) != (a[i + 1] >> 32)) continue;
+        if (i > 0 && (a[i - 1] >> 32) == (x >> 32)) continue;
+        uint32_t e = i + 2;
+        while (e < n && (a[e] >> 32) == (x >> 32)) ++e;
+        for (uint32_t p = i + 1; p < e; ++p) {
+            const unsigned long long k = a[p];
+            uint32_t q = p;
+            while (q > i && a[q - 1] > k) {
+                a[q] = a[q - 1];
+                --q;
+            }
+            a[q] = k;
+        }
+    }
+}
+
+template <int THREADS>
+__device__ __forceinline__ int sort_warps(uint32_t n) {
+    return static_cast<int>(min(static_cast<uint32_t>(THREADS / 32), max(1u, (n + 127u) / 128u)));
+}
+
+template <int THREADS, int KEYS, bool BALLOT>
+__device__ __forceinline__ void sort_slice(const unsigned long long* __restrict__ src, unsigned long long* a, SliceSortSmem<THREADS>& s,
+                                           uint32_t n) {
+    static_assert(THREADS >= 256 && THREADS % 32 == 0, "scan_digits needs a thread per digit");
+    constexpr int kPerLane = KEYS / THREADS;
+    const int lane = threadIdx.x & 31, warp = threadIdx.x >> 5;
+    const int aw = sort_warps<THREADS>(n);
+    const uint32_t seg = ((n + aw - 1) / aw + 31u) & ~31u;
+    const uint32_t w0 = min(n, warp * seg), w1 = min(n, w0 + seg);
+    for (uint32_t i = threadIdx.x; i < n; i += THREADS) a[i] = src[i];
+    for (int shift = 32; shift < 64; shift += 8) {
+        for (int i = threadIdx.x; i < aw * 256; i += THREADS) (&s.cnt[0][0])[i] = 0u;
+        if (threadIdx.x == 0) s.flag = 0;
+        __syncthreads();
+        unsigned long long k[kPerLane];
+#pragma unroll
+        for (int u = 0; u < kPerLane; ++u) {
+            const uint32_t i = w0 + u * 32 + lane;
+            k[u] = i < w1 ? a[i] : 0ull;
+            if (i < w1) atomicAdd(&s.cnt[warp][static_cast<uint32_t>(k[u] >> shift) & 255u], 1u);
+        }
+        __syncthreads();
+        if (scan_digits(s.cnt, s.tot, &s.flag, aw, n)) continue;
+#pragma unroll
+        for (int u = 0; u < kPerLane; ++u) {
+            if (w0 + u * 32 >= w1) break;
+            const bool have = w0 + u * 32 + lane < w1;
+            const uint32_t slot = rank_key<BALLOT>(s.cnt[warp], k[u], shift, have);
+            if (have) a[slot] = k[u];
+        }
+        __syncthreads();
+    }
+    fix_equal_depth_runs<THREADS>(a, n);
+    __syncthreads();
+}
+
+}
+
+}
```
